# KlabCMU/KinPoly

Hardware: AMD Instinct MI355X
Metric: env-steps/sec (whole node) at 4096 envs/GPU, 69-DoF SMPL (higher is better)
Workload: dtype f32

## Files before the change

### include/kinpoly_sim.h

```cpp
#ifndef KINPOLY_SIM_H
#define KINPOLY_SIM_H
#include <stdint.h>
#ifdef __cplusplus
extern "C" {
#endif

typedef struct kp_model kp_model;
typedef struct kp_sim kp_sim;

#define KP_NQ 76
#define KP_NV 75
#define KP_NU 69
#define KP_NBODY 24
#define KP_CC_OBS_DIM 784
#define KP_AR_OBS_DIM 105
#define KP_AR_OBS_DIM_NO_ACTION 101
#define KP_KIN_ACTION_DIM 80
#define KP_CC_ACTION_DIM 75

kp_model* kp_model_load(const char* kpm_path);
int kp_model_compile(const char* xml_path, const char* uhc_yml_path, const char* out_kpm_path);
kp_model* kp_model_load_xml(const char* xml_path, const char* uhc_yml_path);
void kp_model_free(kp_model*);
int kp_model_set_option(kp_model*, const char* name, double value);
double kp_model_get_option(const kp_model*, const char* name);

kp_sim* kp_sim_create(const kp_model*, int n_envs, int device_id, void* hip_stream);
void kp_sim_destroy(kp_sim*);
int kp_sim_n_envs(const kp_sim*);

int kp_sim_set_stream(kp_sim*, void* hip_stream);

const uint32_t* kp_sim_status_device(kp_sim*);

int kp_sim_contacts(kp_sim*, float* out_host);

int kp_sim_mass_matrix(kp_sim*, float* M, float* bias);

int kp_sim_set_state(kp_sim*, const float* qpos, const float* qvel, const uint8_t* env_mask);

int kp_sim_set_target(kp_sim*, const float* target_qpos, const uint8_t* env_mask);

int kp_sim_set_objects(kp_sim*, const float* obj_qpos, const uint8_t* env_mask);

int kp_sim_fk(kp_sim*, int n_rows, const float* qpos, float* qpos_out, float* wbpos, float* wbquat, float* bquat, float* body_com);

int kp_sim_pose_contacts(kp_sim*, int n_rows, const float* xpos, const float* xquat, const float* obj_qpos, float pen_margin,
                         float* pen, int32_t* ncon, uint32_t* hits);

int kp_model_hull_planes(const kp_model*, float* planes4, int32_t* adr);

typedef struct { float figure[4][3], object[3], floor[2][3], sky[3], zfar; } kp_render_style;
void kp_render_style_default(kp_render_style*);

int kp_sim_render(kp_sim*, int n_rows, int n_fig, const float* xpos, const float* xquat, const float* obj_qpos, const float* camera, int camera_rows,
                  int width, int height, const kp_render_style* style, int32_t* geom, float* depth, uint8_t* rgba);

int kp_sim_render_ego(kp_sim*, int n_rows, int n_fig, const float* xpos, const float* xquat, const float* obj_qpos, const float* camera,
                      const float* xpos_b, const float* xquat_b, const float* obj_qpos_b, const float* camera_b, int camera_rows, int width, int height,
                      int hide_body, const kp_render_style* style, int grid_x, int grid_y,
                      int32_t* geom, float* depth, uint8_t* rgba, float* flow, uint8_t* ok, float* cells);

int kp_sim_fk_backward(kp_sim*, int n_rows, const float* qpos, const float* wbpos, const float* wbquat, const float* grad_wbpos, float* grad_qpos);

int kp_sim_step_ctrl(kp_sim*, const float* cc_action, int n_substeps, const uint8_t* env_mask);

int kp_sim_step_kin(kp_sim*, const float* kin_action, float* next_qpos);

int kp_sim_step_head(kp_sim*, const float* kin_action);

int kp_sim_obs_cc(kp_sim*, float* out, const float* zf_mean, const float* zf_std, float clip);

int kp_sim_obs_cc_ex(kp_sim*, float* out, const float* zf_mean, const float* zf_std, float clip, const float* phase);
int kp_sim_cc_obs_dim(const kp_sim*);

typedef struct {
    int T;
    const float* head_pose;
    const float* head_vels;
    const float* obj_head_relative_poses;
    const float* action_one_hot;
    const float* gt_bquat;
    const float* gt_wbpos;
    const float* obj_qpos;
    const int32_t* cur_t;
    const int32_t* row;
} kp_ctx;

int kp_sim_step_begin(kp_sim*);

int kp_sim_obs_ar(kp_sim*, const kp_ctx* ctx, float* out);
int kp_sim_ar_obs_dim(const kp_sim*);

typedef struct {
    float w_hp, w_hq, w_p, w_jp, w_act_p, w_act_v;
    float k_hp, k_hq, k_p, k_jp, k_act_p, k_act_v;
    float dt;
    float body_diff_thresh;
    float body_diff_gt_thresh;
    int use_gt_term;
} kp_reward_cfg;
int kp_sim_term_reward(kp_sim*, const kp_ctx* ctx, const kp_reward_cfg* cfg, float* reward, float* info, uint8_t* fail, float* diffs);

int kp_sim_post_step(kp_sim*, const kp_ctx* ctx, const kp_reward_cfg* cfg, int32_t* cur_t, const int32_t* row_len, int env_episode_len,
                     float* reward, float* info, uint8_t* fail, float* diffs, uint8_t* done, uint8_t* end, float* percent, int32_t* done_count, float* obj7);

typedef struct {
    float w_hp, w_hq, w_p, w_v, w_e;
    float k_hp, k_hq, k_p, k_v, k_e;
    float dt, body_diff_thresh, body_diff_gt_thresh;
    int use_gt_term;
    const float* b_diffw;
} kp_reward_cfg_v2;
int kp_sim_term_reward_v2(kp_sim*, const kp_ctx* ctx, const kp_reward_cfg_v2* cfg, float* reward, float* info, uint8_t* fail, float* diffs);
int kp_sim_post_step_v2(kp_sim*, const kp_ctx* ctx, const kp_reward_cfg_v2* cfg, int32_t* cur_t, const int32_t* row_len, int env_episode_len,
                        float* reward, float* info, uint8_t* fail, float* diffs, uint8_t* done, uint8_t* end, float* percent, int32_t* done_count, float* obj7);

int kp_sim_reset_rows(kp_sim*, const float* init_qpos, const float* init_qvel, const int32_t* row, const uint8_t* env_mask, int32_t* cur_t, int set_target,
                      float* aux_rows, int aux_cols, const float* row_obj_qpos, const float* row_action_one_hot, float* obj7);

int kp_pool_advance(int n, int n_slots, const uint8_t* done, int32_t* head, int32_t* ahead, int32_t* row, void* hip_stream);

typedef struct {
    int n, T, t, ctx_T;
    const float* obs; const uint8_t* fresh; const float* qpos; const float* ctx_qpos; const int32_t* row; const int32_t* cur_t; const int32_t* row_len; const float* row_meta;
    float* states; uint8_t* episode_start; float* curr_qpos; float* gt_target_qpos; float* meta;
} kp_record_pre;
typedef struct {
    int n, T, t; float fr_num;
    const float* action; const float* reward; const uint8_t* fail; const uint8_t* done; const float* percent; const float* c_info;
    const float* obs; const float* qpos; const float* cc_action; const float* cc_state; const float* meta;
    float* actions; float* rewards; uint8_t* fails; uint8_t* dones; float* percents; float* c_infos;
    float* next_states; float* res_qpos; float* cc_actions; float* cc_states; float* v_metas;
} kp_record_post;
int kp_rollout_record_pre(const kp_record_pre*, void* hip_stream);
int kp_rollout_record_post(const kp_record_post*, void* hip_stream);
int kp_rollout_record_pre_w(const kp_record_pre*, int obs_dim, void* hip_stream);
int kp_rollout_record_post_w(const kp_record_post*, int obs_dim, void* hip_stream);

int kp_gae(int n_envs, int T, const float* rewards, const float* masks, const float* values, float gamma, float tau,
           float* advantages, float* returns, void* hip_stream);
int kp_gae_bootstrap(int n_envs, int T, const float* rewards, const float* masks, const float* values, const float* last_values,
                     float gamma, float tau, float* advantages, float* returns, void* hip_stream);

int kp_mcp_compose(int n, int K, int A, const float* logits, const float* prim, const float* noise, int noise_stride, const float* stdv, float* out, void* hip_stream);

int kp_kin_advance(int n, const float* qpos, const float* kin_action, float dt, float* next_qpos, float* qvel_fd, void* hip_stream);

int kp_mcp_tail(int n, int K, int J, int A, const float* h2, const float* b2, const float* w3, int ldw, const float* b3, const float* logits, const float* noise,
                int noise_stride, const float* stdv, float* out, void* hip_stream);

int kp_gru_cell_step(int n, int H, int D, const float* gi, const float* gh, const float* b_ih, const float* b_hh, const float* h_in, const float* state,
                     float* h_out, float* xcat, void* hip_stream);

// ... 168 lines not shown
```

### kinpoly_amd/csrc/kp_obs_kernels.hpp

```cpp
#pragma once
#include "kp_quat.hpp"

namespace kp {

__global__ void k_step_kin(int n, const float* __restrict__ qpos, const float* __restrict__ act, float* __restrict__ next_qpos, float dt) {
    int e = blockIdx.x * blockDim.x + threadIdx.x;
    if (e >= n) return;
    const float* q = qpos + (size_t)e * D_NQ;
    const float* a = act + (size_t)e * 80;
    float* o = next_qpos + (size_t)e * D_NQ;
    Q4 rot = Q4{q[3], q[4], q[5], q[6]};
    Q4 hq = q_heading(rot);
    V3 linv = q_mul_vec(hq, v3(a[74], a[75], a[76]));
    o[0] = q[0] + linv.x * dt; o[1] = q[1] + linv.y * dt;
    o[2] = a[0];
    V3 angv = q_mul_vec(rot, v3(a[77], a[78], a[79]));
    Q4 nr = qmul(q_from_expmap(dt * angv), rot);
    o[3] = nr.w; o[4] = nr.x; o[5] = nr.y; o[6] = nr.z;
    for (int j = 0; j < D_NU; j++) o[7 + j] = a[5 + j];
}

__global__ void k_kin_advance(int n, const float* __restrict__ qpos, const float* __restrict__ act, float dt, float* __restrict__ next_qpos, float* __restrict__ qvel) {
    int e = blockIdx.x * blockDim.x + threadIdx.x;
    if (e >= n) return;
    const float* q = qpos + (size_t)e * D_NQ;
    const float* a = act + (size_t)e * 80;
    float* o = next_qpos + (size_t)e * D_NQ;
    float* v = qvel + (size_t)e * D_NV;
    const Q4 rot = Q4{q[3], q[4], q[5], q[6]};
    const Q4 hq = q_heading(rot);
    const V3 linv = q_mul_vec(hq, v3(a[74], a[75], a[76]));
    const float nx = q[0] + linv.x * dt, ny = q[1] + linv.y * dt, nz = a[0];
    const V3 angv = q_mul_vec(rot, v3(a[77], a[78], a[79]));
    Q4 nr = qmul(q_from_expmap(dt * angv), rot);
    const float nn = sqrtf(nr.w * nr.w + nr.x * nr.x + nr.y * nr.y + nr.z * nr.z);
    nr = Q4{nr.w / nn, nr.x / nn, nr.y / nn, nr.z / nn};
    o[0] = nx; o[1] = ny; o[2] = nz; o[3] = nr.w; o[4] = nr.x; o[5] = nr.y; o[6] = nr.z;
    const float idt = 1.0f / dt;
    v[0] = (nx - q[0]) * idt; v[1] = (ny - q[1]) * idt; v[2] = (nz - q[2]) * idt;
    const float c2 = rot.w * rot.w + rot.x * rot.x + rot.y * rot.y + rot.z * rot.z;
    const Q4 qrel = qmul(nr, Q4{rot.w / c2, -rot.x / c2, -rot.y / c2, -rot.z / c2});
    float sn = sqrtf(qrel.x * qrel.x + qrel.y * qrel.y + qrel.z * qrel.z);
    const V3 ev = dt * angv;
    const bool small = !(sn > 0.0f) || (ev.x == 0.0f && ev.y == 0.0f && ev.z == 0.0f);
    sn = fmaxf(sn, 1e-30f);
    const V3 axis = small ? v3(1.f, 0.f, 0.f) : v3(qrel.x / sn, qrel.y / sn, qrel.z / sn);
    float angle = small ? 0.0f : 2.0f * atan2f(sn, qrel.w);
    if (angle > KP_PI) angle -= KP_2PI;
    if (angle < -KP_PI) angle += KP_2PI;
    const V3 rv = (angle * idt) * axis;
    const float cn = sqrtf(c2);
    const float qw = rot.w / cn;
    const V3 u = v3(-rot.x / cn, -rot.y / cn, -rot.z / cn);
    const V3 t = 2.0f * cross(u, rv);
    const V3 wv = rv + qw * t + cross(u, t);
    v[3] = wv.x; v[4] = wv.y; v[5] = wv.z;
    for (int j = 0; j < D_NU; j++) { const float nj = a[5 + j]; o[7 + j] = nj; v[6 + j] = (nj - q[7 + j]) * idt; }
}

struct TargetBufs { float *qpos, *wbpos, *wbquat, *bquat, *com; };
struct KinStep { const float *act, *xpos, *xquat; float *prev_bquat, *prev_hpos; float dt; };
__global__ __launch_bounds__(256) void k_target_fk(int n, const float* __restrict__ tq, const uint8_t* __restrict__ mask, TargetBufs B,
                                                    const float* __restrict__ body_pos, const float* __restrict__ body_ipos, const int8_t* __restrict__ parent,
                                                    const uint8_t* __restrict__ depth, KinStep K = KinStep{nullptr, nullptr, nullptr, nullptr, nullptr, 0.f}) {
    __shared__ float sq[4][80], swq[4][D_NB * 4], swp[4][D_NB * 3];
    const int w = threadIdx.x >> 6, lane = threadIdx.x & 63;
    const int e = blockIdx.x * 4 + w;
    const bool live = e < n && !(mask && !mask[e]);
    if (!__syncthreads_or(live)) return;
    if (live) {
        const float* q = tq + (size_t)e * D_NQ;
        if (K.act) {
            const float* a = K.act + (size_t)e * 80;
            if (lane < D_NB) {
                const Q4 r = lane == 0 ? Q4{q[3], q[4], q[5], q[6]} : q_euler_sxyz(q[7 + 3 * (lane - 1)], q[8 + 3 * (lane - 1)], q[9 + 3 * (lane - 1)]);
                float* o = K.prev_bquat + ((size_t)e * D_NB + lane) * 4;
                o[0] = r.w; o[1] = r.x; o[2] = r.y; o[3] = r.z;
                if (lane == 13) {
                    for (int k = 0; k < 3; k++) K.prev_hpos[(size_t)e * 7 + k] = K.xpos[(size_t)e * 72 + 39 + k];
                    for (int k = 0; k < 4; k++) K.prev_hpos[(size_t)e * 7 + 3 + k] = K.xquat[(size_t)e * 96 + 52 + k];
                }
            }
            if (lane == 32) {
                const Q4 rot = Q4{q[3], q[4], q[5], q[6]};
                const V3 linv = q_mul_vec(q_heading(rot), v3(a[74], a[75], a[76]));
                const V3 angv = q_mul_vec(rot, v3(a[77], a[78], a[79]));
                const Q4 nr = qmul(q_from_expmap(K.dt * angv), rot);
                sq[w][0] = q[0] + linv.x * K.dt; sq[w][1] = q[1] + linv.y * K.dt; sq[w][2] = a[0];
                sq[w][3] = nr.w; sq[w][4] = nr.x; sq[w][5] = nr.y; sq[w][6] = nr.z;
            }
            for (int j = lane; j < D_NU; j += 64) sq[w][7 + j] = a[5 + j];
        } else {
            for (int i = lane; i < D_NQ; i += 64) sq[w][i] = q[i];
        }
    }
    __syncthreads();
    const int b = lane;
    Q4 wqb = Q4{1.f, 0.f, 0.f, 0.f}, lq = wqb, bq = wqb;
    V3 pos = v3(0.f, 0.f, 0.f);
    int dep = 99, p = 0;
    if (live && b < D_NB) {
        dep = depth[b]; p = parent[b] < 0 ? 0 : parent[b];
        const float* q = sq[w];
        if (b == 0) {
            Q4 rq = Q4{q[3], q[4], q[5], q[6]};
            const float rn = sqrtf(rq.w * rq.w + rq.x * rq.x + rq.y * rq.y + rq.z * rq.z);
            rq = Q4{rq.w / rn, rq.x / rn, rq.y / rn, rq.z / rn};
            wqb = rq; bq = rq; pos = v3(q[0], q[1], q[2]);
        } else {
            const float* ang = q + 7 + 3 * (b - 1);
            lq = q_euler_rzyx(ang[0], ang[1], ang[2]);
            bq = q_euler_sxyz(ang[0], ang[1], ang[2]);
        }
    }
    for (int lev = 0; lev < D_NLEV; lev++) {
        if (dep == lev) {
            if (b > 0) {
                const Q4 pq = Q4{swq[w][4 * p], swq[w][4 * p + 1], swq[w][4 * p + 2], swq[w][4 * p + 3]};
                pos = q_mul_vec(pq, ld3(body_pos + 3 * b)) + ld3(swp[w] + 3 * p);
                wqb = qmul(pq, lq);
            }
            swq[w][4 * b] = wqb.w; swq[w][4 * b + 1] = wqb.x; swq[w][4 * b + 2] = wqb.y; swq[w][4 * b + 3] = wqb.z;
            st3(swp[w] + 3 * b, pos);
        }
        __syncthreads();
    }
    if (live && b < D_NB) {
        if (B.bquat) { float* o = B.bquat + (size_t)e * 96 + 4 * b; o[0] = bq.w; o[1] = bq.x; o[2] = bq.y; o[3] = bq.z; }
        if (B.wbpos) st3(B.wbpos + (size_t)e * 72 + 3 * b, pos);
        if (B.wbquat) { float* o = B.wbquat + (size_t)e * 96 + 4 * b; o[0] = wqb.w; o[1] = wqb.x; o[2] = wqb.y; o[3] = wqb.z; }
        if (B.com) st3(B.com + (size_t)e * 72 + 3 * b, q_mul_vec(wqb, ld3(body_ipos + 3 * b)) + pos);
    }
    if (live && B.qpos) {
        float* oq = B.qpos + (size_t)e * D_NQ;
        for (int i = lane; i < D_NQ; i += 64) oq[i] = (i >= 3 && i < 7) ? swq[w][i - 3] : sq[w][i];
    }
}

__global__ __launch_bounds__(256) void k_fk_wbpos_grad(int n, const float* __restrict__ qpos, const float* __restrict__ wbpos, const float* __restrict__ wbquat,
                                                        const float* __restrict__ gw, float* __restrict__ gq, const int8_t* __restrict__ parent,
                                                        const uint8_t* __restrict__ subtree) {
    __shared__ float sp[4][D_NB * 3], sg[4][D_NB * 3];
    const int w = threadIdx.x >> 6, b = threadIdx.x & 63;
    const int e = blockIdx.x * 4 + w;
    const bool live = e < n;
    if (live && b < D_NB) {
        st3(sp[w] + 3 * b, ld3(wbpos + (size_t)e * 72 + 3 * b));
        st3(sg[w] + 3 * b, ld3(gw + (size_t)e * 72 + 3 * b));
    }
    __syncthreads();
    if (!live || b >= D_NB) return;
    const V3 pb = ld3(sp[w] + 3 * b);
    V3 F = v3(0.f, 0.f, 0.f), M = v3(0.f, 0.f, 0.f);
    const int nb = subtree[b];
    for (int j = b + 1; j < b + nb; j++) {
        const V3 g = ld3(sg[w] + 3 * j);
        F = F + g; M = M + cross(ld3(sp[w] + 3 * j) - pb, g);
    }
    const float* q = qpos + (size_t)e * D_NQ;
    float* o = gq + (size_t)e * D_NQ;
    if (b == 0) {
        st3(o, F + ld3(sg[w]));
        const float qn = sqrtf(q[3] * q[3] + q[4] * q[4] + q[5] * q[5] + q[6] * q[6]);
        const float* uq = wbquat + (size_t)e * 96;
        const Q4 G = qmul(Q4{0.f, 2.f * M.x, 2.f * M.y, 2.f * M.z}, Q4{uq[0], uq[1], uq[2], uq[3]});
        o[3] = G.w / qn; o[4] = G.x / qn; o[5] = G.y / qn; o[6] = G.z / qn;
    } else {
        const int p = parent[b];
        const float* pq = wbquat + (size_t)e * 96 + 4 * p;
        float R[9];
        q_matrix(Q4{pq[0], pq[1], pq[2], pq[3]}, R);
        const float tz = q[7 + 3 * (b - 1)], ty = q[8 + 3 * (b - 1)];
        float sz, cz, sy, cy;
        sincosf(tz, &sz, &cz); sincosf(ty, &sy, &cy);
        const V3 az = mulmat(R, v3(0.f, 0.f, 1.f));
        const V3 ay = mulmat(R, v3(-sz, cz, 0.f));
        const V3 ax = mulmat(R, v3(cz * cy, sz * cy, -sy));
        o[7 + 3 * (b - 1)] = dot(az, M); o[8 + 3 * (b - 1)] = dot(ay, M); o[9 + 3 * (b - 1)] = dot(ax, M);
    }
}

__global__ void k_bquat(int n, const float* __restrict__ qpos, float* __restrict__ out) {
    int t = blockIdx.x * blockDim.x + threadIdx.x;
    if (t >= n * D_NB) return;
    int e = t / D_NB, b = t - e * D_NB;
    const float* q = qpos + (size_t)e * D_NQ;
    Q4 r;
    if (b == 0) r = Q4{q[3], q[4], q[5], q[6]};
    else r = q_euler_sxyz(q[7 + 3 * (b - 1)], q[8 + 3 * (b - 1)], q[9 + 3 * (b - 1)]);
    float* o = out + (size_t)t * 4;
    o[0] = r.w; o[1] = r.x; o[2] = r.y; o[3] = r.z;
}

struct ObsCcArgs {
    int n;
    const float *qpos, *qvel, *xpos, *xquat, *xipos;
    const float *t_qpos, *t_wbpos, *t_wbquat, *t_com;
    float br_inv[4];
    const float *zf_mean, *zf_std; float clip;
    float* out;
};
template <int V, bool VROOT, bool HEAD, bool DEHEAD, bool PHASE>
struct ObsCcLayout {
    static constexpr int LV = VROOT ? 6 : 75;
    static constexpr int D = V == 0 ? (HEAD ? 1 : 0) + 74 + LV + 69 + (PHASE ? 1 : 0) : 229 + LV + (V == 1 ? 4 : 2) * 72 + 2 * 96;
};
template <int V, bool VROOT, bool HEAD, bool DEHEAD, bool PHASE>
__device__ __forceinline__ void obs_cc_body(const ObsCcArgs& A, const float* __restrict__ phase) {
    using L = ObsCcLayout<V, VROOT, HEAD, DEHEAD, PHASE>;
    constexpr int LV = L::LV, D = L::D;
    __shared__ float ob[D];
    const int e = blockIdx.x, tid = threadIdx.x;
    if (e >= A.n) return;
    const float* qpos = A.qpos + (size_t)e * D_NQ;
    const float* qvel = A.qvel + (size_t)e * D_NV;
    const float* tq = A.t_qpos + (size_t)e * D_NQ;
    const Q4 rq = Q4{qpos[3], qpos[4], qpos[5], qpos[6]};
    if constexpr (V == 0) {
        constexpr int H = HEAD ? 1 : 0, K = H + 74 + LV;
        if (tid == 0) {
            if (HEAD) ob[0] = heading_angle(rq);
            const Q4 r = DEHEAD ? qmul(q_inverse(q_heading(rq)), rq) : rq;
            ob[H] = qpos[2]; ob[H + 1] = r.w; ob[H + 2] = r.x; ob[H + 3] = r.y; ob[H + 4] = r.z;
            const V3 v = q_tmul_vec(rq, v3(qvel[0], qvel[1], qvel[2]));
            ob[H + 74] = v.x; ob[H + 75] = v.y; ob[H + 76] = v.z;
            if (PHASE) ob[K + 69] = phase[e];
        }
        for (int i = tid; i < 69; i += 64) { ob[H + 5 + i] = qpos[7 + i]; ob[K + i] = tq[7 + i]; }
        for (int i = tid; i < LV - 3; i += 64) ob[H + 77 + i] = qvel[3 + i];
    } else {
        constexpr int P = 229 + LV, NJ = V == 1 ? 4 : 2, Q = P + 72 * NJ;
        const Q4 binv = Q4{A.br_inv[0], A.br_inv[1], A.br_inv[2], A.br_inv[3]};
        const Q4 crq = qmul(rq, binv);
        const Q4 hq = q_heading(crq);
        const Q4 trq = qmul(Q4{tq[3], tq[4], tq[5], tq[6]}, binv);
        const V3 root = v3(qpos[0], qpos[1], qpos[2]);
        if (tid == 0) {
            ob[0] = hq.w; ob[1] = hq.x; ob[2] = hq.y; ob[3] = hq.z;
            Q4 dh = qmul(q_inverse(hq), crq);
            ob[78] = qpos[2]; ob[79] = dh.w; ob[80] = dh.x; ob[81] = dh.y; ob[82] = dh.z;
            Q4 dq = qmul(trq, q_inverse(crq));
            ob[152] = tq[2] - qpos[2]; ob[153] = dq.w; ob[154] = dq.x; ob[155] = dq.y; ob[156] = dq.z;
            V3 v = q_tmul_vec(crq, q_tmul_vec(rq, v3(qvel[0], qvel[1], qvel[2])));
            ob[226] = v.x; ob[227] = v.y; ob[228] = v.z;
            float rel_h = heading_angle(trq) - heading_angle(crq);
            if (rel_h > KP_PI) rel_h -= KP_2PI;
            if (rel_h < -KP_PI) rel_h += KP_2PI;
            ob[P - 3] = rel_h;
            V3 rp = q_tmul_vec(crq, v3(trq.w, trq.x, trq.y) - root);
            ob[P - 2] = rp.x; ob[P - 1] = rp.y;
        }
        for (int i = tid; i < 74; i += 64) ob[4 + i] = tq[2 + i];
        for (int i = tid; i < 69; i += 64) { ob[83 + i] = qpos[7 + i]; ob[157 + i] = tq[7 + i] - qpos[7 + i]; }
        for (int i = tid; i < LV - 3; i += 64) ob[229 + i] = qvel[3 + i];
        if (tid < D_NB) {
            const int b = tid;
            const float* xp = A.xpos + (size_t)e * 72 + 3 * b;
            const float* xi = A.xipos + (size_t)e * 72 + 3 * b;
            const float* xq = A.xquat + (size_t)e * 96;
            V3 cj = ld3(xp), ci = ld3(xi);
            V3 tj = ld3(A.t_wbpos + (size_t)e * 72 + 3 * b), tc = ld3(A.t_com + (size_t)e * 72 + 3 * b);
            V3 p1 = q_tmul_vec(crq, cj - root), p2 = q_tmul_vec(crq, tj - cj), p3 = q_tmul_vec(crq, ci - root), p4 = q_tmul_vec(crq, tc - ci);
            ob[P + b] = p1.x; ob[P + 24 + b] = p1.y; ob[P + 48 + b] = p1.z;
            ob[P + 72 + b] = p2.x; ob[P + 96 + b] = p2.y; ob[P + 120 + b] = p2.z;
            if (V == 1) {
                ob[P + 144 + b] = p3.x; ob[P + 168 + b] = p3.y; ob[P + 192 + b] = p3.z;
                ob[P + 216 + b] = p4.x; ob[P + 240 + b] = p4.y; ob[P + 264 + b] = p4.z;
            }
            const float* twq = A.t_wbquat + (size_t)e * 96 + 4 * b;
            Q4 tqt = Q4{twq[0], twq[1], twq[2], twq[3]};
            Q4 cq = (xq[0] == 0.f) ? tqt : Q4{xq[4 * b], xq[4 * b + 1], xq[4 * b + 2], xq[4 * b + 3]};
            Q4 r1 = qmul(q_inverse(hq), cq), r2 = qmul(q_inverse(cq), tqt);
            float* o1 = ob + Q + 4 * b; o1[0] = r1.w; o1[1] = r1.x; o1[2] = r1.y; o1[3] = r1.z;
            float* o2 = ob + Q + 96 + 4 * b; o2[0] = r2.w; o2[1] = r2.x; o2[2] = r2.y; o2[3] = r2.z;
        }
    }
    __syncthreads();
    for (int i = tid; i < D; i += 64) {
        float v = ob[i];
        if (A.zf_mean) {
            v = (v - A.zf_mean[i]) / (A.zf_std[i] + 1e-8f);
            if (A.clip > 0.f) v = fminf(fmaxf(v, -A.clip), A.clip);
        }
        A.out[(size_t)e * D + i] = v;
    }
}
template <int V, bool VROOT, bool HEAD, bool DEHEAD, bool PHASE>
__global__ __launch_bounds__(64) void k_obs_cc(ObsCcArgs A, const float* __restrict__ phase) { obs_cc_body<V, VROOT, HEAD, DEHEAD, PHASE>(A, phase); }
__global__ __launch_bounds__(64) void k_obs_cc_uhc(ObsCcArgs A) { obs_cc_body<1, false, false, false, false>(A, nullptr); }

}
```

### kinpoly_amd/csrc/kp_rollout_kernels.hpp

```cpp
#pragma once
#include "kp_obs_kernels.hpp"
#include "kp_obs_ar_row.hpp"

namespace kp {

__device__ __forceinline__ int obj_action_start(const float* one_hot) {
    if (!one_hot) return -1;
    int a = -1;
    for (int k = 0; k < 4; k++) if (a < 0 && one_hot[k] != 0.f) a = k;
    return a < 0 ? -1 : (a == 0 ? 0 : (a == 1 ? 7 : (a == 2 ? 21 : 28)));
}

template <bool VEL, bool HEAD, bool ACTION>
__global__ __launch_bounds__(256) void k_obs_ar(int n, CtxDev C, const float* __restrict__ qpos, const float* __restrict__ qvel,
                                                 const float* __restrict__ xpos, const float* __restrict__ xquat, float* __restrict__ out) {
    const int l = threadIdx.x & 31, e = blockIdx.x * 8 + (threadIdx.x >> 5);
    if (e >= n) return;
    obs_ar_row<VEL, HEAD, ACTION>(C, e, l, qpos, qvel, xpos, xquat, out + (size_t)e * ObsArLayout<VEL, HEAD, ACTION>::D);
}

template <bool ACTION>
__global__ void k_obs_ar_thread(int n, CtxDev C, const float* __restrict__ qpos, const float* __restrict__ xpos, const float* __restrict__ xquat,
                                float* __restrict__ out) {
    int e = blockIdx.x * blockDim.x + threadIdx.x;
// ... 88 lines not shown
    float pq = 0.f, pp = 0.f, pg = 0.f, vel2 = 0.f, bd = 0.f, bgd = 0.f;
    if (b < D_NB) {
        const Q4 cb = b == 0 ? Q4{q[3], q[4], q[5], q[6]} : q_euler_sxyz(q[7 + 3 * (b - 1)], q[8 + 3 * (b - 1)], q[9 + 3 * (b - 1)]);
        const float* tb = t_bquat + (size_t)e * 96 + 4 * b;
        if constexpr (RV == 1) pq = quat_norm_v2(qmul(cb, q_inverse(Q4{tb[0], tb[1], tb[2], tb[3]})));
        const V3 x = ld3(xp + 3 * b);
        const V3 dpos = x - ld3(t_wbpos + (size_t)e * 72 + 3 * b);
        pp = sqrtf(dot(dpos, dpos));
        const float wgt = diffw ? diffw[b] : 1.0f;
        bd = wgt * pp;
        const V3 dg = x - ld3(gtw + 3 * b);
        bgd = wgt * sqrtf(dot(dg, dg));
        const Q4 g = Q4{gtb[4 * b], gtb[4 * b + 1], gtb[4 * b + 2], gtb[4 * b + 3]};
        const Q4 gpv = Q4{gtp[4 * b], gtp[4 * b + 1], gtp[4 * b + 2], gtp[4 * b + 3]};
        if constexpr (RV == 1) pg = quat_norm_v2(qmul(g, q_inverse(cb)));
        else {
            const Q4 qd = qmul(cb, q_inverse(g));
            const float pa = atan2f(sqrtf(qd.x * qd.x + qd.y * qd.y + qd.z * qd.z), qd.w) * W.b_diffw[b];
            pq = pa * pa;
            pg = dot(dg, dg);
        }
        const float* pb = prev_bquat + (size_t)e * 96 + 4 * b;
        constexpr float rot_eps = RV == 1 ? 1e-8f : 1e-6f;
        const V3 cv = (1.0f / W.dt) * rot_from_quat(qmul(cb, q_inverse(Q4{pb[0], pb[1], pb[2], pb[3]})), rot_eps);
        const V3 gv = (1.0f / W.dt) * rot_from_quat(qmul(g, q_inverse(gpv)), rot_eps);
        const V3 dv = cv - gv;
        vel2 = dot(dv, dv);
    }
#pragma unroll
    for (int m = 16; m >= 1; m >>= 1) {
        pq += __shfl_xor(pq, m, 32); pp += __shfl_xor(pp, m, 32); pg += __shfl_xor(pg, m, 32);
        vel2 += __shfl_xor(vel2, m, 32); bd += __shfl_xor(bd, m, 32); bgd += __shfl_xor(bgd, m, 32);
    }
    if (b != 0 || !valid) return;
    const float* xq = xquat + (size_t)e * 96;
    const float* hp = C.head_pose + (C.r(e) * C.T + t) * 7;
    const V3 hd = ld3(xp + 39) - ld3(hp);
    const float hp_r = expf(-W.k_hp * dot(hd, hd));
    const Q4 hq = qmul(Q4{xq[52], xq[53], xq[54], xq[55]}, q_inverse(Q4{hp[3], hp[4], hp[5], hp[6]}));
    const float hqd = quat_norm_v2(hq);
    const float hq_r = expf(-W.k_hq * hqd * hqd);
    if constexpr (RV == 1) {
        pq *= (1.0f / 24.0f); pp *= (1.0f / 24.0f); pg *= (1.0f / 24.0f);
        const float p_r = expf(-W.k_p * pq * pq), jp_r = expf(-W.k_jp * pp * pp);
        const float gt_r = expf(-W.k_act_p * pg), av_r = expf(-W.k_act_v * vel2);
        reward[e] = W.w_hp * hp_r + W.w_hq * hq_r + W.w_p * p_r + W.w_jp * jp_r + W.w_act_p * gt_r + W.w_act_v * av_r;
        float* inf = info + (size_t)e * 6;
        inf[0] = hp_r; inf[1] = hq_r; inf[2] = p_r; inf[3] = jp_r; inf[4] = gt_r; inf[5] = av_r;
    } else {
        const float p_r = expf(-W.k_p * pq), v_r = expf(-W.k_v * vel2), e_r = expf(-W.k_e * pg);
        reward[e] = W.w_hp * hp_r + W.w_hq * hq_r + W.w_p * p_r + W.w_v * v_r + W.w_e * e_r;
        float* inf = info + (size_t)e * 6;
        inf[0] = hp_r; inf[1] = hq_r; inf[2] = p_r; inf[3] = v_r; inf[4] = e_r; inf[5] = 0.f;
    }
    const bool failed = (bd > W.thresh) || (W.use_gt && bgd > W.gt_thresh) || !(bd == bd);
    fail[e] = failed;
    diffs[2 * e] = bd; diffs[2 * e + 1] = bgd;
    if (POST) {
        const int clen = PS.row_len[C.r(e)];
        const bool ended = t_now >= (clen < PS.episode_len ? clen : PS.episode_len);
        PS.cur_t[e] = t_now;
        PS.end[e] = ended; PS.done[e] = failed || ended;
        PS.percent[e] = (float)t_now / (float)clen;
        if (PS.done_count && (failed || ended)) atomicAdd(PS.done_count, 1);
        if (PS.obj7) {
            const int st = obj_action_start(C.action_one_hot + C.r(e) * 4);
            if (st >= 0) for (int k = 0; k < 7; k++) PS.obj7[(size_t)e * 7 + k] = PS.sim_obj_qpos[(size_t)e * 35 + st + k];
        }
    }
}

__global__ void k_reset_rows(int n, const float* __restrict__ init_qpos, const float* __restrict__ init_qvel, const int* __restrict__ row,
                             const uint8_t* __restrict__ mask, int* __restrict__ cur_t, float* __restrict__ qpos, float* __restrict__ qvel,
                             float* __restrict__ qpos_d, float* __restrict__ qvel_d, float* __restrict__ warm, float* __restrict__ aux_rows, int aux_cols) {
    const int e = blockIdx.x, i = threadIdx.x;
    if (e >= n || (mask && !mask[e])) return;
    for (int c = i; c < aux_cols; c += 128) aux_rows[(size_t)e * aux_cols + c] = 0.f;
    const size_t r = row ? (size_t)row[e] : (size_t)e;
    if (i < D_NQ) { const float v = init_qpos[r * D_NQ + i]; qpos[(size_t)e * D_NQ + i] = v; qpos_d[(size_t)e * D_NQ + i] = v; }
    if (i < D_NV) { const float v = init_qvel[r * D_NV + i]; qvel[(size_t)e * D_NV + i] = v; qvel_d[(size_t)e * D_NV + i] = v; warm[(size_t)e * D_NV + i] = 0.f; }
    if (i == 0 && cur_t) cur_t[e] = 0;
}

__global__ void k_pool_advance(int n, int n_slots, const uint8_t* __restrict__ done, int* __restrict__ head, int* __restrict__ ahead, int* __restrict__ row) {
    const int e = blockIdx.x * blockDim.x + threadIdx.x;
    if (e >= n || !done[e]) return;
    const int a = ahead[e];
    ahead[e] = a - 1;
    if (a <= 0) return;
    int h = head[e] + 1;
    if (h >= n_slots) h = 0;
    head[e] = h;
    row[e] = h * n + e;
}

struct RecordPre {
    int n, T, t, ctx_T, obs_dim;
    const float* obs; const uint8_t* fresh; const float* qpos; const float* ctx_qpos; const int* row; const int* cur_t; const int* row_len; const float* row_meta;
    float* states; uint8_t* episode_start; float* curr_qpos; float* gt_target_qpos; float* meta;
};
struct RecordPost {
    int n, T, t, obs_dim; float fr_num;
    const float* action; const float* reward; const uint8_t* fail; const uint8_t* done; const float* percent; const float* c_info;
    const float* obs; const float* qpos; const float* cc_action; const float* cc_state; const float* meta_t;
    float* actions; float* rewards; uint8_t* fails; uint8_t* dones; float* percents; float* c_infos;
    float* next_states; float* res_qpos; float* cc_actions; float* cc_states; float* v_metas;
};

__device__ __forceinline__ void copy_row(float* __restrict__ dst, const float* __restrict__ src, int dim) {
    for (int i = threadIdx.x; i < dim; i += blockDim.x) dst[i] = src[i];
}

__global__ void k_record_pre(RecordPre R) {
    const int e = blockIdx.x;
    if (e >= R.n) return;
    const size_t at = (size_t)e * R.T + R.t;
    if (R.states) copy_row(R.states + at * R.obs_dim, R.obs + (size_t)e * R.obs_dim, R.obs_dim);
    if (R.curr_qpos) copy_row(R.curr_qpos + at * 76, R.qpos + (size_t)e * 76, 76);
    const int r = R.row ? R.row[e] : e;
    if (R.gt_target_qpos) {
        int f = R.cur_t[e] + 1;
        const int last = R.row_len[r];
        if (f > last) f = last;
        copy_row(R.gt_target_qpos + at * 76, R.ctx_qpos + ((size_t)r * R.ctx_T + f) * 76, 76);
    }
    if (threadIdx.x == 0) {
        if (R.episode_start) R.episode_start[at] = R.fresh[e];
        if (R.meta) { R.meta[at * 2] = R.row_meta[(size_t)r * 2]; R.meta[at * 2 + 1] = R.row_meta[(size_t)r * 2 + 1]; }
    }
}

__global__ void k_record_post(RecordPost R) {
    const int e = blockIdx.x;
    if (e >= R.n) return;
    const size_t at = (size_t)e * R.T + R.t;
    if (R.actions) copy_row(R.actions + at * 80, R.action + (size_t)e * 80, 80);
    if (R.next_states) copy_row(R.next_states + at * R.obs_dim, R.obs + (size_t)e * R.obs_dim, R.obs_dim);
    if (R.res_qpos) copy_row(R.res_qpos + at * 76, R.qpos + (size_t)e * 76, 76);
    if (R.cc_actions) copy_row(R.cc_actions + at * 75, R.cc_action + (size_t)e * 75, 75);
    if (R.cc_states) copy_row(R.cc_states + at * 784, R.cc_state + (size_t)e * 784, 784);
    if (R.c_infos && threadIdx.x < 6) R.c_infos[at * 6 + threadIdx.x] = R.c_info[(size_t)e * 6 + threadIdx.x];
    if (threadIdx.x == 0) {
        if (R.rewards) R.rewards[at] = R.reward[e];
        if (R.fails) R.fails[at] = R.fail[e];
        if (R.dones) R.dones[at] = R.done[e];
        if (R.percents) R.percents[at] = R.percent[e];
        if (R.v_metas) { R.v_metas[at * 3] = R.meta_t[at * 2]; R.v_metas[at * 3 + 1] = R.meta_t[at * 2 + 1]; R.v_metas[at * 3 + 2] = R.fr_num; }
    }
}

__global__ void k_gae(int n, int T, const float* __restrict__ rewards, const float* __restrict__ masks, const float* __restrict__ values,
                      const float* __restrict__ last_values, float gamma, float tau, float* __restrict__ adv, float* __restrict__ ret) {
    int e = blockIdx.x * blockDim.x + threadIdx.x;
    if (e >= n) return;
    float prev_v = last_values ? last_values[e] : 0.f, prev_a = 0.f;
    for (int t = T - 1; t >= 0; t--) {
        size_t i = (size_t)e * T + t;
        float m = masks[i], v = values[i];
        float delta = rewards[i] + gamma * prev_v * m - v;
        float a = delta + gamma * tau * prev_a * m;
        adv[i] = a; ret[i] = v + a;
        prev_v = v; prev_a = a;
    }
}

__global__ void k_mcp_compose(int n, int K, int A, const float* __restrict__ logits, const float* __restrict__ prim, const float* __restrict__ noise,
// ... 53 lines not shown
```

### kinpoly_amd/csrc/kp_sim.hip

```cpp
#include <hip/hip_runtime.h>

#include <climits>
#include <cmath>
#include <algorithm>
#include <array>
#include <cstdlib>
#include <cstring>
#include <cstdio>
#include <unistd.h>
#include <string>
#include <utility>
#include <vector>

#include "../../include/kinpoly_sim.h"
#include "kp_model.hpp"
#include "kp_obs_kernels.hpp"
#include "kp_rollout_kernels.hpp"
#include "kp_policy_kernels.hpp"
#include "kp_step_kernel.hpp"
#include "kp_readout.hpp"
#include "kp_pose_contacts.hpp"
#include "kp_render.hpp"
#include "kp_render_ego.hpp"
#include "kp_takes.hpp"
#include "kp_kin_tape.hpp"
#include "kp_obs_ctx.hpp"

namespace {
thread_local std::string g_err;
int fail(const std::string& m) { g_err = m; return -1; }
#define HIP_OK(expr) do { hipError_t e_ = (expr); if (e_ != hipSuccess) return fail(std::string(#expr) + ": " + hipGetErrorString(e_)); } while (0)
#define HIP_OK_NULL(expr) do { hipError_t e_ = (expr); if (e_ != hipSuccess) { fail(std::string(#expr) + ": " + hipGetErrorString(e_)); return nullptr; } } while (0)
int launched() { HIP_OK(hipGetLastError()); return 0; }
}

struct kp_model {
    kp::HostModel h;
    int contact = 1, limits = 1, stale = 1, solver_iter = 100, threads = 64, dynamic_objects = 1, lpt_order = -1, substeps_per_job = 4, queue_slots = 0, job_taper = 1, queue_fence = 1, queue_heavy = 160, queue_prio = -1, queue_late = -1, job_auto = 1, lean_queue = 1, lean_adaptive = 1, lds_pad = 0, lean_cap = kp::EnvLdsLean::MAXCON;
    double warm_extrap = -1.0;
    int planemesh_max = 3; double planemesh_tol = 0.3;
    int ar_obs_action = 1;
    int ar_obs_vel = 0, ar_obs_head = 1;
    int cc_obs_v = 1, cc_obs_vel_root = 0, cc_obs_heading = 0, cc_obs_deheading = 0, cc_obs_phase = 0;
    int cc_action_v = 1, cc_rfc = 1, cc_meta_pd = 0;
    int actuation = 1;
    double solver_tol = 1e-8, gravity_z = -9.81, gravity_x = 0.0, gravity_y = 0.0;
};

struct StateRows {
    float *qpos = nullptr, *qvel = nullptr, *qpos_d = nullptr, *qvel_d = nullptr, *warm = nullptr, *warm2 = nullptr, *warm3 = nullptr;
    float *xpos = nullptr, *xquat = nullptr, *xipos = nullptr, *prev_bquat = nullptr, *prev_hpos = nullptr;
    int* diag = nullptr;
};
struct JobQueue {
    int* order = nullptr; unsigned* cost = nullptr;
    unsigned *jobq = nullptr, *jobctr = nullptr, *ovfq = nullptr;
    float* spd_next = nullptr;
    int wave_slots = 2048;
    int nsub = -1, layout = -1;
};
struct OverflowReadback {
    unsigned* host = nullptr; hipEvent_t ev[2] = {nullptr, nullptr}; bool pending[2] = {false, false};
    long lean_off_until = -1; int fallbacks = 0;
    unsigned last = 0;
};
struct ObjectRows {
    float *qpos = nullptr, *geoms = nullptr;
    float *qvel = nullptr, *warm = nullptr, *warm2 = nullptr;
    signed char* slot = nullptr;
    int* ngeom = nullptr;
    const float* d_geoms = nullptr; const float* d_mass = nullptr; int n_geoms = 0, n_obj = 0;
    bool on = false;
};
struct Timing {
    hipEvent_t ev0 = nullptr, ev1 = nullptr, last0 = nullptr, last1 = nullptr;
    std::vector<hipEvent_t> ring;
    int ring_used = 0;
    bool ring_on = false, timed = false;
};

struct RenderTables {
    const float* planes = nullptr; const int32_t* adr = nullptr;
    float* partial = nullptr; size_t partial_n = 0;
};

struct InvDynScratch {
    float* buf = nullptr; size_t rows = 0;
};

struct MarkerScratch {
    static constexpr int MAXK = 1024, WORDS = 4 * MAXK + 25;
    void* buf = nullptr;
    std::vector<uint32_t> host;
};

struct kp_sim {
    const kp_model* model = nullptr;
    int n = 0, device = 0;
    int ar_obs_vel = 0, ar_obs_head = 1, ar_obs_action = 1;
    int ar_obs_dim = KP_AR_OBS_DIM;
    int cc_obs_v = 1, cc_obs_vel_root = 0, cc_obs_heading = 0, cc_obs_deheading = 0, cc_obs_phase = 0, cc_obs_dim = KP_CC_OBS_DIM;
    kp::XcArgs xc{KP_CC_ACTION_DIM, 0, 1, 0};
    bool xc_on = false;
    hipStream_t stream = nullptr;
    std::vector<void*> allocs;
    kp::DevTables T{};
    kp::Params P{};
    float* diffw = nullptr;
    StateRows st;
    kp::TargetBufs tgt{};
    JobQueue q;
    OverflowReadback ovf;
    ObjectRows obj;
    RenderTables rd;
    InvDynScratch idyn;
    MarkerScratch mk;
    Timing tm;
    long launch_index = 0;
    int last_nsub = 15;
    unsigned long long* prof = nullptr;
    bool prof_noted = false;
    float* dbg_contacts = nullptr;
    int32_t* uhc_stage = nullptr;
};

struct kp_takes {
    const kp_model* model = nullptr;
    int device = 0;
    kp::TakeTables L{};
    float* obj = nullptr;
    std::vector<int32_t> off;
    std::vector<void*> allocs;
};

namespace {

template <typename T, typename S>
const T* upload(kp_sim* s, const std::vector<S>& src, bool* ok) {
    std::vector<T> tmp(src.size());
    for (size_t i = 0; i < src.size(); i++) tmp[i] = (T)src[i];
    void* d = nullptr;
    if (hipMalloc(&d, std::max<size_t>(sizeof(T) * tmp.size(), 16)) != hipSuccess) { *ok = false; return nullptr; }
    s->allocs.push_back(d);
    if (hipMemcpy(d, tmp.data(), sizeof(T) * tmp.size(), hipMemcpyHostToDevice) != hipSuccess) { *ok = false; return nullptr; }
    return (const T*)d;
}

float* dalloc(kp_sim* s, size_t count, bool* ok) {
    void* d = nullptr;
    if (hipMalloc(&d, sizeof(float) * count) != hipSuccess) { *ok = false; return nullptr; }
    s->allocs.push_back(d);
    hipMemset(d, 0, sizeof(float) * count);
    return (float*)d;
}

bool build_tables(kp_sim* s) {
    const kp::HostModel& m = s->model->h;
    using namespace kp;
    bool ok = true;
    auto& T = s->T;
    T.body_pos = upload<float>(s, m.body_pos, &ok); T.body_ipos = upload<float>(s, m.body_ipos, &ok);
    T.body_mass = upload<float>(s, m.body_mass, &ok); T.body_inertia = upload<float>(s, m.body_inertia, &ok);
    T.body_rbound = upload<float>(s, m.body_rbound, &ok); T.mesh_rbound = upload<float>(s, m.mesh_rbound, &ok);
    std::vector<double> invw(NB), liminvw(NU), lo(NU), hi(NU);
    for (int b = 0; b < NB; b++) invw[b] = m.body_invweight0[2 * b];
    for (int j = 0; j < NU; j++) { liminvw[j] = m.dof_invweight0[6 + j]; lo[j] = m.jnt_range[2 * j]; hi[j] = m.jnt_range[2 * j + 1]; }
    T.body_invw = upload<float>(s, invw, &ok); T.lim_invw = upload<float>(s, liminvw, &ok);
    T.jnt_lo = upload<float>(s, lo, &ok); T.jnt_hi = upload<float>(s, hi, &ok);
    T.dof_armature = upload<float>(s, m.dof_armature, &ok);
    T.kp = upload<float>(s, m.kp, &ok); T.kd = upload<float>(s, m.kd, &ok); T.tlim = upload<float>(s, m.torque_lim, &ok);
    T.ascale = upload<float>(s, m.a_scale, &ok);
    s->diffw = const_cast<float*>(upload<float>(s, m.body_diffw, &ok));
    T.verts = upload<float>(s, m.verts, &ok);
    T.vert_adr = upload<uint16_t>(s, m.vert_adr, &ok);
    T.vert_nbr_adr = upload<uint16_t>(s, m.vert_nbr_adr, &ok); T.vert_nbr = upload<uint8_t>(s, m.vert_nbr, &ok);
    T.dof_body = upload<uint8_t>(s, m.dof_body, &ok);
    T.body_parent = upload<int8_t>(s, m.body_parent, &ok); T.body_depth = upload<uint8_t>(s, m.body_depth, &ok);
    T.body_subtree = upload<uint8_t>(s, m.body_subtree, &ok); T.jnt_limited = upload<uint8_t>(s, m.jnt_limited, &ok);
    for (int b = 1; b < NB; b++) {
        if (m.body_parent[b] >= b) return false;
        for (int j = 0; j < 3; j++) if (m.dof_body[6 + 3 * (b - 1) + j] != b) return false;
    }
    for (int b = 0; b < NB; b++)
        for (int k = b + 1; k < NB; k++) {
            bool desc = false;
            for (int p = m.body_parent[k]; p >= 0; p = m.body_parent[p]) if (p == b) desc = true;
            if (desc != (k < b + m.body_subtree[b])) return false;
        }
    std::vector<int> lev_start(D_NLEV + 2, 0), lev_body;
    for (int lev = 0; lev <= D_NLEV; lev++) {
        lev_start[lev] = (int)lev_body.size();
        for (int b = 0; b < NB; b++) if (m.body_depth[b] == lev) lev_body.push_back(b);
    }
    lev_start[D_NLEV + 1] = (int)lev_body.size();
    if ((int)lev_body.size() != NB || lev_start[D_NLEV] != NB) return false;
// ... 62 lines not shown
    P.mu = (float)o[OPT_FRIC]; P.margin = (float)o[OPT_MARGIN];
    P.pm_max = s->model->planemesh_max; P.pm_tol = (float)s->model->planemesh_tol;
    P.scale = (float)(1.0 / (o[OPT_MEANINERTIA] * (o.size() > OPT_NV_FULL ? o[OPT_NV_FULL] : NV)));
    P.rfc_scale = (float)o[OPT_RFC_SCALE]; P.rfc_lim = (float)o[OPT_RFC_LIM];
    double bn = o[OPT_BR_W] * o[OPT_BR_W] + o[OPT_BR_X] * o[OPT_BR_X] + o[OPT_BR_Y] * o[OPT_BR_Y] + o[OPT_BR_Z] * o[OPT_BR_Z];
    P.br_inv[0] = (float)(o[OPT_BR_W] / bn); P.br_inv[1] = (float)(-o[OPT_BR_X] / bn);
    P.br_inv[2] = (float)(-o[OPT_BR_Y] / bn); P.br_inv[3] = (float)(-o[OPT_BR_Z] / bn);
    P.tol = (float)s->model->solver_tol; P.max_iter = s->model->solver_iter;
    P.contact = s->model->contact; P.limits = s->model->limits; P.stale = s->model->stale; P.actuation = s->model->actuation;
    return ok;
}

int job_schedule(int nsub, int spj, int taper, int* sizes) {
    int parts = 0, rem = nsub, size = spj;
    while (rem > 0 && parts < 16) {
        int take = parts == 15 ? rem : std::min(rem, size);
        if (rem - take > 0 && rem - take < spj) take = rem;
        sizes[parts++] = take; rem -= take;
        size += taper;
    }
    std::reverse(sizes, sizes + parts);
    return parts;
}

bool lean_eligible(const kp_sim& s) { return !s.obj.on && s.model->lean_queue && s.model->threads == 64 && s.P.stale && !s.xc_on; }

int envs_per_cu(size_t lds_bytes, int reg_cap) { return std::min(reg_cap, 128 / (int)((lds_bytes + 1279) / 1280)); }

int poll_overflow(kp_sim* s) {
    for (int k = 0; k < 2; k++) {
        if (!s->ovf.pending[k]) continue;
        const hipError_t e = hipEventQuery(s->ovf.ev[k]);
        if (e == hipErrorNotReady) continue;
        s->ovf.pending[k] = false;
        if (e != hipSuccess) return fail(std::string("hipEventQuery(ovf_ev): ") + hipGetErrorString(e));
        s->ovf.last = s->ovf.host[k];
        if ((size_t)s->ovf.host[k] * 64 > (size_t)s->n) { s->ovf.lean_off_until = s->launch_index + 64; s->ovf.fallbacks++; }
    }
    return 0;
}

enum Layout { FULL = 0, OBJECTS = 1, LEAN = 2 };
struct StepPlan {
    bool queue, lpt;
    bool prof_per_env;
    Layout layout;
    int threads, slots, parts, sizes[16], queue_prio, queue_late, ovf_grid;
    size_t lds;
};

StepPlan plan_step(const kp_sim& s, int nsub, bool capturing) {
    const kp_model& m = *s.model;
    StepPlan p{};
    bool lean = lean_eligible(s);
    if (lean && nsub > 0 && s.ovf.host && !capturing && m.lean_adaptive && s.launch_index < s.ovf.lean_off_until) lean = false;
    p.layout = s.obj.on ? OBJECTS : lean ? LEAN : FULL;
    p.threads = m.threads;
    p.lpt = nsub > 0 && (m.lpt_order > 0 || (m.lpt_order < 0 && s.obj.on));
    const size_t lds = s.obj.on ? sizeof(kp::EnvLdsObj) : sizeof(kp::EnvLds);
    size_t lds_q = lean ? sizeof(kp::EnvLdsLean) : lds;
    if (m.lds_pad > 0) lds_q = std::max(lds_q, (size_t)m.lds_pad);
    p.slots = m.queue_slots > 0 ? m.queue_slots : s.q.wave_slots / 8 * envs_per_cu(lds_q, lean ? 12 : 8);
    const bool lean_auto = lean && m.job_auto;
    const int spj = lean_auto ? 5 : m.substeps_per_job, taper = lean_auto ? 0 : m.job_taper;
    if (spj > 0 && nsub > 0) {
        p.parts = job_schedule(nsub, spj, taper, p.sizes);
        if (const char* e = std::getenv("KP_JOB_SCHEDULE")) {
            int tmp[16], np = 0, sum = 0;
            for (const char* c = e; *c && np < 16;) { tmp[np] = std::atoi(c); sum += tmp[np++]; while (*c && *c != ',') c++; if (*c) c++; }
            if (sum == nsub) { p.parts = np; std::copy(tmp, tmp + np, p.sizes); }
        }
    }
    const int resident_full = s.q.wave_slots / 8 * envs_per_cu(lds, 8);
    const bool queue = nsub > 0 && p.parts > 1 && m.threads == 64 && s.n > std::min(p.slots, resident_full) && s.n <= 0xFFFFFF;
    p.queue = queue && !s.prof; p.prof_per_env = queue && s.prof;
    p.lds = p.queue ? lds_q : lds;
    p.queue_prio = m.queue_prio >= 0 ? m.queue_prio : (lean ? 3 : 0);
    p.queue_late = m.queue_late >= 0 ? m.queue_late : (lean ? 1 : 0);
    p.ovf_grid = std::min(std::min(s.n, resident_full), std::max(128, 2 * (int)std::min<unsigned>(s.ovf.last, 1u << 20)));
    return p;
}

template <int NT, bool OBJ>
void launch_per_env(const kp_sim* s, const kp::StepArgs& A, int nsub, size_t lds) {
    if (nsub > 0 && s->prof && s->xc_on) hipLaunchKernelGGL((kp::kp_step_kernel_xc<NT, OBJ, true>), dim3(s->n), dim3(NT), lds, s->stream, A, s->xc);
    else if (nsub > 0 && s->prof) hipLaunchKernelGGL((kp::kp_step_kernel<NT, OBJ, true>), dim3(s->n), dim3(NT), lds, s->stream, A);
    else if (nsub > 0 && s->xc_on) hipLaunchKernelGGL((kp::kp_step_kernel_xc<NT, OBJ>), dim3(s->n), dim3(NT), lds, s->stream, A, s->xc);
    else if (nsub > 0) hipLaunchKernelGGL((kp::kp_step_kernel<NT, OBJ>), dim3(s->n), dim3(NT), lds, s->stream, A);
    else hipLaunchKernelGGL((kp::kp_forward_kernel<NT, OBJ>), dim3(s->n), dim3(NT), lds, s->stream, A);
}

int timing_begin(kp_sim* s, hipEvent_t* e0, hipEvent_t* e1) {
    Timing& t = s->tm;
    *e0 = t.ev0; *e1 = t.ev1;
    if (t.ring_on && t.ring_used < 4096) {
        if ((int)t.ring.size() < 2 * (t.ring_used + 1)) {
            hipEvent_t a, b;
            HIP_OK(hipEventCreate(&a)); HIP_OK(hipEventCreate(&b));
            t.ring.push_back(a); t.ring.push_back(b);
        }
        *e0 = t.ring[2 * t.ring_used]; *e1 = t.ring[2 * t.ring_used + 1];
        t.ring_used++;
    }
    HIP_OK(hipEventRecord(*e0, s->stream));
    return 0;
}
int timing_end(kp_sim* s, hipEvent_t e0, hipEvent_t e1) {
    HIP_OK(hipEventRecord(e1, s->stream));
    s->tm.last0 = e0; s->tm.last1 = e1; s->tm.timed = true;
    return 0;
}

kp::StepArgs step_args(const kp_sim* s, const StepPlan& p, int nsub, const float* action, const uint8_t* mask, const float* base_qpos) {
    const kp_model& m = *s->model;
    const StateRows& st = s->st; const ObjectRows& o = s->obj; const JobQueue& q = s->q;
    kp::StepArgs A{};
    A.T = s->T; A.P = s->P; A.n_envs = s->n; A.n_substeps = nsub;
    A.qpos = st.qpos; A.qvel = st.qvel; A.qpos_d = st.qpos_d; A.qvel_d = st.qvel_d; A.warm = st.warm; A.warm2 = st.warm2; A.warm3 = st.warm3;
    A.target_qpos = base_qpos ? base_qpos : s->tgt.qpos; A.action = action; A.env_mask = mask;
    A.xpos = st.xpos; A.xquat = st.xquat; A.xipos = st.xipos; A.diag = st.diag; A.prof = s->prof; A.dbg_contacts = s->dbg_contacts;
    A.geoms = o.geoms; A.ngeom = o.ngeom; A.obj_slot = o.slot; A.obj_qpos = o.qpos; A.obj_qvel = o.qvel; A.obj_warm = o.warm; A.obj_warm2 = o.warm2;
    A.warm_extrap = m.warm_extrap < 0 ? (o.on ? 0.75f : 0.f) : (float)m.warm_extrap;
    A.order = p.lpt ? q.order : nullptr; A.order_valid = p.lpt; A.cost = q.cost;
    A.jobq = q.jobq; A.jobctr = q.jobctr; A.ovfq = q.ovfq; A.spd_next = q.spd_next; A.lean_cap = m.lean_cap;
    A.n_parts = p.queue ? p.parts : 1; A.queue_fence = m.queue_fence; A.queue_heavy = m.queue_heavy; A.queue_prio = p.queue_prio; A.queue_late = p.queue_late;
    for (int k = 0; p.queue && k < p.parts; k++) (k < 8 ? A.part_sub_lo : A.part_sub_hi) |= (unsigned long long)(p.sizes[k] & 255) << (8 * (k & 7));
    return A;
}

int launch_queue(kp_sim* s, const StepPlan& p, kp::StepArgs& A, int nsub, bool capturing) {
    JobQueue& q = s->q;
    if (nsub != q.nsub || (int)p.layout != q.layout) {
        HIP_OK(hipMemsetAsync(q.jobctr + 32, 0, 2 * sizeof(unsigned), s->stream));
        q.nsub = nsub; q.layout = (int)p.layout;
    }
    const unsigned total = (unsigned)s->n * (unsigned)p.parts;
    hipLaunchKernelGGL(kp::k_queue_init, dim3((total + 255) / 256), dim3(256), 0, s->stream, s->n, total, q.jobq, q.jobctr, A.order);
    A.order = nullptr;
    if (s->xc_on && p.layout == OBJECTS) hipLaunchKernelGGL((kp::kp_step_queue_kernel_xc<true>), dim3(p.slots), dim3(64), p.lds, s->stream, A, s->xc);
    else if (s->xc_on) hipLaunchKernelGGL((kp::kp_step_queue_kernel_xc<false>), dim3(p.slots), dim3(64), p.lds, s->stream, A, s->xc);
    else if (p.layout == OBJECTS) hipLaunchKernelGGL((kp::kp_step_queue_kernel<true>), dim3(p.slots), dim3(64), p.lds, s->stream, A);
    else if (p.layout == FULL) hipLaunchKernelGGL((kp::kp_step_queue_kernel<false>), dim3(p.slots), dim3(64), p.lds, s->stream, A);
    else {
        hipLaunchKernelGGL((kp::kp_step_queue_kernel<false, true>), dim3(p.slots), dim3(64), p.lds, s->stream, A);
        hipLaunchKernelGGL(kp::kp_step_overflow_kernel, dim3(p.ovf_grid), dim3(64), sizeof(kp::EnvLds), s->stream, A);
        const int k = (int)(s->launch_index & 1);
        if (s->ovf.host && !capturing && !s->ovf.pending[k]) {
            HIP_OK(hipMemcpyAsync(s->ovf.host + k, q.jobctr + 64, sizeof(unsigned), hipMemcpyDeviceToHost, s->stream));
            HIP_OK(hipEventRecord(s->ovf.ev[k], s->stream));
            s->ovf.pending[k] = true;
        }
    }
    return 0;
}

int launch_step(kp_sim* s, const float* action, int nsub, const uint8_t* mask, bool time_it, const float* base_qpos = nullptr) {
    const int threads = s->model->threads;
    if (s->obj.on && threads != 64) return fail("object contact needs threads_per_env = 64");
    if (threads != 64 && threads != 128 && threads != 256) return fail("threads_per_env must be 64, 128 or 256");
    hipStreamCaptureStatus cap = hipStreamCaptureStatusNone;
    const bool capturing = hipStreamIsCapturing(s->stream, &cap) == hipSuccess && cap != hipStreamCaptureStatusNone;
    time_it = time_it && !capturing;
    hipEvent_t e0 = nullptr, e1 = nullptr;
    if (time_it && timing_begin(s, &e0, &e1)) return -1;
    if (nsub > 0 && s->ovf.host && !capturing && lean_eligible(*s) && poll_overflow(s)) return -1;
    const StepPlan p = plan_step(*s, nsub, capturing);
    if (nsub > 0) { s->launch_index++; s->last_nsub = nsub; }
    if (p.prof_per_env && !s->prof_noted) {
        std::fprintf(stderr, "kp_sim: KP_PROFILE=1: the job-queue kernels carry no phase profiler; this handle's control steps run one workgroup per env "
                             "(kp_step_kernel), whose profiling instantiation fills kp_sim_phase_cycles\n");
        s->prof_noted = true;
    }
    kp::StepArgs A = step_args(s, p, nsub, action, mask, base_qpos);
    if (p.lpt) hipLaunchKernelGGL(kp::k_lpt_order, dim3(1), dim3(1024), 0, s->stream, s->n, s->q.cost, s->q.order);
    if (p.queue) { if (launch_queue(s, p, A, nsub, capturing)) return -1; }
    else if (s->obj.on) launch_per_env<64, true>(s, A, nsub, p.lds);
    else if (p.threads == 64) launch_per_env<64, false>(s, A, nsub, p.lds);
    else if (p.threads == 128) launch_per_env<128, false>(s, A, nsub, p.lds);
    else launch_per_env<256, false>(s, A, nsub, p.lds);
    HIP_OK(hipGetLastError());
    return time_it ? timing_end(s, e0, e1) : 0;
}

void launch_target_fk(const kp_sim* s, int n, const float* tq, const uint8_t* mask, const kp::TargetBufs& B,
                      const kp::KinStep& K = kp::KinStep{nullptr, nullptr, nullptr, nullptr, nullptr, 0.f}) {
    hipLaunchKernelGGL(kp::k_target_fk, dim3((n + 3) / 4), dim3(256), 0, s->stream, n, tq, mask, B, s->T.body_pos, s->T.body_ipos, s->T.body_parent, s->T.body_depth, K);
}

}

extern "C" {

const char* kp_last_error(void) { return g_err.c_str(); }
const char* kp_version(void) { return "kinpoly_sim 0.1 (gfx950)"; }

kp_model* kp_model_load(const char* path) {
    kp_model* m = new kp_model();
    if (!kp::load_kpm(path, m->h)) { fail("kp_model_load: " + m->h.error); delete m; return nullptr; }
    m->gravity_z = m->h.opt[kp::OPT_GZ]; m->gravity_x = m->h.opt[kp::OPT_GX]; m->gravity_y = m->h.opt[kp::OPT_GY];
    m->solver_tol = m->h.opt[kp::OPT_SOLVER_TOL];
    m->solver_iter = (int)m->h.opt[kp::OPT_SOLVER_ITER];
    if (m->solver_iter < 1) m->solver_iter = 100;
    m->planemesh_max = (int)m->h.planemesh[0]; m->planemesh_tol = m->h.planemesh[1];
    return m;
}
void kp_model_free(kp_model* m) { delete m; }

static int cc_action_width(int rfc, int meta) { return 69 + 6 * rfc + (meta == 1 ? 30 : meta == 2 ? 138 : 0); }

static int cc_obs_width(int v, int vel_root, int heading, int phase) {
    const int lv = vel_root ? 6 : 75;
    return v == 0 ? heading + 74 + lv + 69 + phase : 229 + lv + (v == 1 ? 4 : 2) * 72 + 2 * 96;
}

static int ar_obs_width(int vel, int head, int action) { return 74 + 75 * vel + 7 * head + 7 + 13 * head + 4 * action; }
static bool ar_obs_width_known(int d) {
    for (int k = 0; k < 8; k++) if (d == ar_obs_width(k & 1, (k >> 1) & 1, (k >> 2) & 1)) return true;
    return false;
}
#define KP_AR_OBS_WIDTHS "105, 101, 180, 176, 85, 81, 160 or 156"

enum OptRule { O_BOOL, O_TRI, O_INT, O_REAL, O_REAL32, O_ENUM, O_RANGE, O_CLAMP, O_THREADS, O_READ_ONLY };
struct Opt {
    const char* name;
    OptRule rule;
    int kp_model::*i; double kp_model::*d;
    double lo, hi;
    const char* must;
    bool clears_job_auto;
    double (*get)(const kp_model&);
};
constexpr double INF = HUGE_VAL;
#define OPT_I(name, rule, member, ...) Opt{name, rule, &kp_model::member, nullptr, __VA_ARGS__}
#define OPT_D(name, rule, member, ...) Opt{name, rule, nullptr, &kp_model::member, __VA_ARGS__}
#define OPT_RO(name, expr) Opt{name, O_READ_ONLY, nullptr, nullptr, 0, 0, nullptr, false, [](const kp_model& m) -> double { return expr; }}
static const Opt OPTIONS[] = {
    OPT_I("contact", O_BOOL, contact), OPT_I("limits", O_BOOL, limits), OPT_I("actuation", O_BOOL, actuation), OPT_I("stale_kinematics", O_BOOL, stale),
    OPT_D("gravity_z", O_REAL, gravity_z), OPT_D("gravity_x", O_REAL, gravity_x), OPT_D("gravity_y", O_REAL, gravity_y),
    OPT_I("solver_iter", O_INT, solver_iter), OPT_D("solver_tol", O_REAL, solver_tol), OPT_I("dynamic_objects", O_BOOL, dynamic_objects),
    OPT_I("planemesh_max", O_RANGE, planemesh_max, 1, 8), OPT_D("planemesh_tol", O_RANGE, planemesh_tol, 0, INF, ">= 0"),
    OPT_I("threads_per_env", O_THREADS, threads, 0, 0, "64, 128 or 256"),
    OPT_D("warm_extrap", O_REAL32, warm_extrap),
    OPT_I("ar_obs_action", O_ENUM, ar_obs_action, 0, 1, "1 (105-d observation with the action one-hot) or 0 (101-d, use_action: false)"),
    OPT_I("ar_obs_vel", O_ENUM, ar_obs_vel, 0, 1, "0 (no velocities) or 1 (use_vel: the 75 qvel follow the pose block)"),
    OPT_I("ar_obs_head", O_ENUM, ar_obs_head, 0, 1, "1 (with the head-tracking blocks) or 0 (use_head: false)"),
    OPT_RO("ar_obs_dim", ar_obs_width(m.ar_obs_vel, m.ar_obs_head, m.ar_obs_action)),
    OPT_I("cc_obs_v", O_ENUM, cc_obs_v, 0, 2, "0 (get_full_obs), 1 (get_full_obs_v1) or 2 (get_full_obs_v2)"),
    OPT_I("cc_obs_vel_root", O_ENUM, cc_obs_vel_root, 0, 1), OPT_I("cc_obs_heading", O_ENUM, cc_obs_heading, 0, 1),
    OPT_I("cc_obs_deheading", O_ENUM, cc_obs_deheading, 0, 1), OPT_I("cc_obs_phase", O_ENUM, cc_obs_phase, 0, 1),
    OPT_RO("cc_obs_dim", m.cc_obs_v == 0 ? cc_obs_width(0, m.cc_obs_vel_root, m.cc_obs_heading, m.cc_obs_phase) : cc_obs_width(m.cc_obs_v, m.cc_obs_vel_root, 0, 0)),
    OPT_I("cc_action_v", O_ENUM, cc_action_v, 0, 1), OPT_I("cc_rfc", O_ENUM, cc_rfc, 0, 1),
    OPT_I("cc_meta_pd", O_ENUM, cc_meta_pd, 0, 2, "0 (none), 1 (meta_pd: by substep) or 2 (meta_pd_joint: by joint)"),
    OPT_RO("cc_action_dim", cc_action_width(m.cc_rfc, m.cc_meta_pd)),
    OPT_RO("n_obj_geoms", (double)(m.h.obj_geoms.size() / 18)),
    OPT_RO("timestep", m.h.opt[kp::OPT_TIMESTEP]),
    OPT_I("lpt_order", O_TRI, lpt_order),
    OPT_I("substeps_per_job", O_RANGE, substeps_per_job, 0, 255, "0 (whole control step per workgroup) .. 255", true),
    OPT_I("job_taper", O_CLAMP, job_taper, 0, 8, nullptr, true),
    OPT_RO("job_auto", m.job_auto),
    OPT_I("queue_slots", O_RANGE, queue_slots, 0, INF, ">= 0 (0 = resident wave slots of the device)"),
    OPT_I("queue_fence", O_BOOL, queue_fence), OPT_I("queue_heavy", O_CLAMP, queue_heavy, 0, INT_MAX),
    OPT_I("queue_late", O_TRI, queue_late), OPT_I("queue_prio", O_CLAMP, queue_prio, -1, 3),
    OPT_I("lean_queue", O_BOOL, lean_queue), OPT_I("lean_adaptive", O_BOOL, lean_adaptive),
    OPT_I("lean_max_contacts", O_RANGE, lean_cap, 0, kp::EnvLdsLean::MAXCON),
    OPT_I("lds_pad", O_RANGE, lds_pad, 0, 65536, "0 .. 65536 bytes"),
    OPT_RO("lds_bytes_per_env", (double)sizeof(kp::EnvLds)), OPT_RO("lds_bytes_per_env_objects", (double)sizeof(kp::EnvLdsObj)),
    OPT_RO("lds_bytes_per_env_lean", (double)sizeof(kp::EnvLdsLean)),
};
#undef OPT_I
#undef OPT_D
#undef OPT_RO
static const Opt* find_option(const char* name) {
    for (const Opt& o : OPTIONS) if (name && !std::strcmp(name, o.name)) return &o;
    return nullptr;
}

int kp_model_set_option(kp_model* m, const char* name, double v) {
    if (!m || !name) return fail("kp_model_set_option: null argument");
    const Opt* o = find_option(name);
    if (!o || o->rule == O_READ_ONLY) return fail(std::string("kp_model_set_option: unknown option ") + name);
    bool ok = true;
    double x = v;
    switch (o->rule) {
        case O_BOOL: x = v != 0; break;
        case O_TRI: x = v < 0 ? -1 : (v != 0); break;
        case O_REAL32: x = (float)v; break;
        case O_ENUM: ok = false; for (int k = 0; k <= (int)o->hi; k++) ok = ok || v == k; break;
        case O_RANGE: ok = !(v < o->lo || v > o->hi); break;
        case O_CLAMP: x = std::max((int)o->lo, std::min((int)o->hi, (int)v)); break;
        case O_THREADS: ok = v == 64 || v == 128 || v == 256; break;
        default: break;
    }
    if (!ok) {
        const std::string must = o->must ? o->must : o->rule == O_ENUM ? "0 or 1" : std::to_string((int)o->lo) + " .. " + std::to_string((int)o->hi);
        return fail(std::string(name) + " must be " + must);
    }
    if (o->i) m->*(o->i) = (int)x; else m->*(o->d) = x;
    if (o->clears_job_auto) m->job_auto = 0;
    return 0;
}
double kp_model_get_option(const kp_model* m, const char* name) {
    const Opt* o = find_option(name);
    if (!m || !o) return NAN;
    return o->get ? o->get(*m) : o->i ? (double)(m->*(o->i)) : m->*(o->d);
}

kp_sim* kp_sim_create(const kp_model* m, int n_envs, int device_id, void* stream) {
    if (!m || n_envs <= 0) { fail("kp_sim_create: bad arguments"); return nullptr; }
    int ndev = 0;
    if (hipGetDeviceCount(&ndev) != hipSuccess || ndev == 0) { fail("kp_sim_create: no HIP device available (the simulator has no CPU fallback)"); return nullptr; }
    HIP_OK_NULL(hipSetDevice(device_id));
    kp_sim* s = new kp_sim();
    s->model = m; s->n = n_envs; s->device = device_id; s->stream = (hipStream_t)stream;
    s->ar_obs_vel = m->ar_obs_vel; s->ar_obs_head = m->ar_obs_head; s->ar_obs_action = m->ar_obs_action;
    s->ar_obs_dim = ar_obs_width(s->ar_obs_vel, s->ar_obs_head, s->ar_obs_action);
    s->cc_obs_v = m->cc_obs_v; s->cc_obs_vel_root = m->cc_obs_vel_root;
    s->cc_obs_heading = m->cc_obs_v == 0 && m->cc_obs_heading; s->cc_obs_deheading = m->cc_obs_v == 0 && m->cc_obs_deheading; s->cc_obs_phase = m->cc_obs_v == 0 && m->cc_obs_phase;
    s->cc_obs_dim = cc_obs_width(s->cc_obs_v, s->cc_obs_vel_root, s->cc_obs_heading, s->cc_obs_phase);
    s->xc = kp::XcArgs{cc_action_width(m->cc_rfc, m->cc_meta_pd), m->cc_action_v == 0, m->cc_rfc, m->cc_meta_pd};
    s->xc_on = m->cc_action_v != 1 || m->cc_rfc != 1 || m->cc_meta_pd != 0;
    bool ok = build_tables(s);
    const size_t N = n_envs;
    StateRows& st = s->st;
    st.qpos = dalloc(s, N * 76, &ok); st.qvel = dalloc(s, N * 75, &ok); st.qpos_d = dalloc(s, N * 76, &ok); st.qvel_d = dalloc(s, N * 75, &ok);
    st.warm = dalloc(s, N * 75, &ok); st.warm2 = dalloc(s, N * 75, &ok); st.warm3 = dalloc(s, N * 75, &ok);
    st.xpos = dalloc(s, N * 72, &ok); st.xquat = dalloc(s, N * 96, &ok); st.xipos = dalloc(s, N * 72, &ok);
    st.prev_bquat = dalloc(s, N * 96, &ok); st.prev_hpos = dalloc(s, N * 7, &ok); st.diag = (int*)dalloc(s, N * 4, &ok);
    s->tgt = kp::TargetBufs{dalloc(s, N * 76, &ok), dalloc(s, N * 72, &ok), dalloc(s, N * 96, &ok), dalloc(s, N * 96, &ok), dalloc(s, N * 72, &ok)};
    JobQueue& q = s->q;
    q.order = (int*)dalloc(s, N, &ok); q.cost = (unsigned*)dalloc(s, N, &ok);
    q.jobq = (unsigned*)dalloc(s, N * 16, &ok); q.jobctr = (unsigned*)dalloc(s, 128, &ok); q.ovfq = (unsigned*)dalloc(s, N, &ok);
    q.spd_next = dalloc(s, N * 80, &ok);
    hipDeviceProp_t prop;
    if (hipGetDeviceProperties(&prop, s->device) == hipSuccess && prop.multiProcessorCount > 0) q.wave_slots = prop.multiProcessorCount * 8;
    ObjectRows& o = s->obj;
    o.qpos = dalloc(s, N * 35, &ok); o.qvel = dalloc(s, N * 30, &ok); o.geoms = dalloc(s, N * kp::D_MAXGEOM * 17, &ok); o.ngeom = (int*)dalloc(s, N, &ok);
    o.warm = dalloc(s, N * 6 * kp::D_MAXOBJ, &ok); o.warm2 = dalloc(s, N * 6 * kp::D_MAXOBJ, &ok); o.slot = (signed char*)dalloc(s, (N * kp::D_MAXOBJ + 3) / 4 + 1, &ok);
    if (!m->h.obj_geoms.empty()) {
        o.d_geoms = upload<float>(s, m->h.obj_geoms, &ok); o.d_mass = upload<float>(s, m->h.obj_mass, &ok);
        o.n_geoms = (int)(m->h.obj_geoms.size() / 18); o.n_obj = (int)m->h.obj_mass.size();
    }
    if (const char* e = std::getenv("KP_PROFILE")) if (e[0] == '1') s->prof = (unsigned long long*)dalloc(s, N * 16, &ok);
    OverflowReadback& v = s->ovf;
    if (hipHostMalloc((void**)&v.host, 2 * sizeof(unsigned), hipHostMallocDefault) != hipSuccess) v.host = nullptr;
    else {
        v.host[0] = v.host[1] = 0u;
        if (hipEventCreateWithFlags(&v.ev[0], hipEventDisableTiming) != hipSuccess || hipEventCreateWithFlags(&v.ev[1], hipEventDisableTiming) != hipSuccess) { hipHostFree(v.host); v.host = nullptr; }
    }
    if (!ok || hipEventCreate(&s->tm.ev0) != hipSuccess || hipEventCreate(&s->tm.ev1) != hipSuccess) {
        fail("kp_sim_create: device allocation / table build failed");
        kp_sim_destroy(s);
        return nullptr;
    }
    return s;
}

void kp_sim_destroy(kp_sim* s) {
    if (!s) return;
    hipSetDevice(s->device);
    hipStreamSynchronize(s->stream);
    for (void* p : s->allocs) hipFree(p);
    if (s->rd.partial) hipFree(s->rd.partial);
    if (s->idyn.buf) hipFree(s->idyn.buf);
    if (s->mk.buf) hipFree(s->mk.buf);
    for (hipEvent_t e : s->tm.ring) hipEventDestroy(e);
    if (s->ovf.host) { hipHostFree(s->ovf.host); for (hipEvent_t e : s->ovf.ev) if (e) hipEventDestroy(e); }
    if (s->tm.ev0) hipEventDestroy(s->tm.ev0);
    if (s->tm.ev1) hipEventDestroy(s->tm.ev1);
    delete s;
}
int kp_sim_n_envs(const kp_sim* s) { return s ? s->n : -1; }

int kp_sim_set_stream(kp_sim* s, void* stream) {
    if (!s) return fail("kp_sim_set_stream: null argument");
    s->stream = (hipStream_t)stream;
    return 0;
}

const uint32_t* kp_sim_status_device(kp_sim* s) { return s ? s->q.jobctr : nullptr; }

int kp_sim_contacts(kp_sim* s, float* out_host) {
    if (!s) return fail("kp_sim_contacts: null argument");
    HIP_OK(hipSetDevice(s->device));
    const size_t count = (size_t)s->n * (1 + kp::D_MAXCON * 9);
    if (!s->dbg_contacts) {
        bool ok = true;
        s->dbg_contacts = dalloc(s, count, &ok);
        if (!ok) return fail("kp_sim_contacts: allocation failed");
        if (out_host) std::memset(out_host, 0, sizeof(float) * count);
        return 0;
    }
    if (!out_host) return 0;
    HIP_OK(hipStreamSynchronize(s->stream));
    HIP_OK(hipMemcpy(out_host, s->dbg_contacts, sizeof(float) * count, hipMemcpyDeviceToHost));
    return 0;
}

int kp_sim_mass_matrix(kp_sim* s, float* M, float* bias) {
    if (!s || (!M && !bias)) return fail("kp_sim_mass_matrix: null argument");
    HIP_OK(hipSetDevice(s->device));
    kp::StepArgs A{};
    A.T = s->T; A.P = s->P; A.n_envs = s->n; A.n_substeps = 0;
    A.qpos_d = s->st.qpos_d; A.qvel_d = s->st.qvel_d;
    hipLaunchKernelGGL(kp::kp_mass_kernel, dim3(s->n), dim3(64), sizeof(kp::EnvLds), s->stream, A, M, bias);
    return launched();
}

__global__ void k_copy_rows(int n, int dim, const float* __restrict__ src, float* __restrict__ dst, float* __restrict__ dst2,
                            const uint8_t* __restrict__ mask) {
    size_t t = (size_t)blockIdx.x * blockDim.x + threadIdx.x;
    if (t >= (size_t)n * dim) return;
    int e = (int)(t / dim);
    if (mask && !mask[e]) return;
    float v = src ? src[t] : 0.f;
    dst[t] = v;
    if (dst2) dst2[t] = v;
}
static void copy_rows(const kp_sim* s, int dim, const float* src, float* dst, float* dst2, const uint8_t* mask) {
    hipLaunchKernelGGL(k_copy_rows, dim3((s->n * dim + 255) / 256), dim3(256), 0, s->stream, s->n, dim, src, dst, dst2, mask);
}

int kp_sim_set_state(kp_sim* s, const float* qpos, const float* qvel, const uint8_t* mask) {
    if (!s || !qpos || !qvel) return fail("kp_sim_set_state: null argument");
    HIP_OK(hipSetDevice(s->device));
    copy_rows(s, 76, qpos, s->st.qpos, s->st.qpos_d, mask);
    copy_rows(s, 75, qvel, s->st.qvel, s->st.qvel_d, mask);
    copy_rows(s, 75, nullptr, s->st.warm, nullptr, mask);
    HIP_OK(hipGetLastError());
    return launch_step(s, nullptr, 0, mask, false);
}

int kp_sim_set_target(kp_sim* s, const float* tq, const uint8_t* mask) {
    if (!s || !tq) return fail("kp_sim_set_target: null argument");
    HIP_OK(hipSetDevice(s->device));
    launch_target_fk(s, s->n, tq, mask, s->tgt);
    return launched();
}

__global__ void k_set_objects(int n, const float* __restrict__ obj_qpos_all, const uint8_t* __restrict__ mask, float* __restrict__ obj_qpos,
                              float* __restrict__ geoms, int* __restrict__ ngeom, const float* __restrict__ og, const float* __restrict__ omass,
                              int n_og, int n_obj, int dynamic, signed char* __restrict__ slot, float* __restrict__ obj_qvel, float* __restrict__ obj_warm,
                              const int* __restrict__ row, const float* __restrict__ one_hot, float* __restrict__ obj7) {
    int e = blockIdx.x * blockDim.x + threadIdx.x;
    if (e >= n) return;
    if (mask && !mask[e]) return;
    int ng = 0, ns = 0;
    const size_t r = row ? (size_t)row[e] : (size_t)e;
    const float* src = obj_qpos_all + r * 35;
// ... 404 lines not shown
        if (!ok) { s->uhc_stage = nullptr; return fail("kp_sim_uhc_assign: allocation failed"); }
    }
    kp::UhcAssignArgs A{};
    if (take_ids) {
        HIP_OK(hipMemcpyAsync(s->uhc_stage, take_ids, sizeof(int32_t) * s->n, hipMemcpyHostToDevice, s->stream));
        A.take_ids = s->uhc_stage;
        if (start) { HIP_OK(hipMemcpyAsync(s->uhc_stage + s->n, start, sizeof(int32_t) * s->n, hipMemcpyHostToDevice, s->stream)); A.start = s->uhc_stage + s->n; }
    }
    A.L = t->L; A.n = s->n; A.keep_t = keep_t; A.obs_v = c->obs_v; A.st = *st; A.mask = mask; A.noise = noise; A.a_ref = c->a_ref;
    A.qpos = s->st.qpos; A.qpos_d = s->st.qpos_d; A.qvel = s->st.qvel; A.qvel_d = s->st.qvel_d; A.warm = s->st.warm;
    A.t_qpos = s->tgt.qpos; A.t_wbpos = s->tgt.wbpos; A.t_wbquat = s->tgt.wbquat; A.t_bquat = s->tgt.bquat; A.t_com = s->tgt.com;
    if (t->obj) {
        ObjectRows& o = s->obj;
        kp::UhcAssignObjArgs B{};
        B.A = A; B.obj_tab = t->obj; B.obj_qpos = o.qpos; B.obj_qvel = o.qvel; B.obj_warm = o.warm; B.geoms = o.geoms; B.ngeom = o.ngeom; B.slot = o.slot;
        B.og = o.d_geoms; B.omass = o.d_mass; B.n_og = o.n_geoms; B.n_obj = o.n_obj;
        B.dynamic = s->model->dynamic_objects && s->T.obj_inertial != nullptr;
        HIP_OK(kp::launch_uhc_assign_obj(B, s->stream));
        o.on = true;
    } else
        HIP_OK(kp::launch_uhc_assign(A, s->stream));
    return launch_step(s, nullptr, 0, mask, false);
}

int kp_sim_step_head(kp_sim* s, const float* act) {
    if (!s || !act) return fail("kp_sim_step_head: null argument");
    HIP_OK(hipSetDevice(s->device));
    launch_target_fk(s, s->n, s->st.qpos, nullptr, s->tgt, kp::KinStep{act, s->st.xpos, s->st.xquat, s->st.prev_bquat, s->st.prev_hpos, 1.0f / 30.0f});
    return launched();
}

int kp_sim_step_kin(kp_sim* s, const float* act, float* next_qpos) {
    if (!s || !act || !next_qpos) return fail("kp_sim_step_kin: null argument");
    HIP_OK(hipSetDevice(s->device));
    hipLaunchKernelGGL(kp::k_step_kin, dim3((s->n + 63) / 64), dim3(64), 0, s->stream, s->n, s->st.qpos, act, next_qpos, 1.0f / 30.0f);
    return launched();
}

static kp::ObsCcArgs obs_cc_args(const kp_sim* s, float* out, const float* zf_mean, const float* zf_std, float clip) {
    kp::ObsCcArgs A;
    A.n = s->n; A.qpos = s->st.qpos; A.qvel = s->st.qvel; A.xpos = s->st.xpos; A.xquat = s->st.xquat; A.xipos = s->st.xipos;
    A.t_qpos = s->tgt.qpos; A.t_wbpos = s->tgt.wbpos; A.t_wbquat = s->tgt.wbquat; A.t_com = s->tgt.com;
    for (int k = 0; k < 4; k++) A.br_inv[k] = s->P.br_inv[k];
    A.zf_mean = zf_mean; A.zf_std = zf_std; A.clip = clip; A.out = out;
    return A;
}

extern "C++" {
using ObsCcLaunch = void (*)(kp_sim*, const kp::ObsCcArgs&, const float*);
template <int V, int I>
static void launch_obs_cc(kp_sim* s, const kp::ObsCcArgs& A, const float* phase) {
    if constexpr (V == 1 && I == 0) hipLaunchKernelGGL(kp::k_obs_cc_uhc, dim3(s->n), dim3(64), 0, s->stream, A);
    else hipLaunchKernelGGL((kp::k_obs_cc<V, (I & 1) != 0, (I & 2) != 0, (I & 4) != 0, (I & 8) != 0>), dim3(s->n), dim3(64), 0, s->stream, A, phase);
}
template <int... I>
static constexpr std::array<ObsCcLaunch, 20> obs_cc_table(std::integer_sequence<int, I...>) {
    return {launch_obs_cc<0, I>..., launch_obs_cc<1, 0>, launch_obs_cc<1, 1>, launch_obs_cc<2, 0>, launch_obs_cc<2, 1>};
}
static constexpr auto OBS_CC = obs_cc_table(std::make_integer_sequence<int, 16>{});
static constexpr int OBS_CC_V1 = 16;
}

int kp_sim_obs_cc(kp_sim* s, float* out, const float* zf_mean, const float* zf_std, float clip) {
    if (!s || !out) return fail("kp_sim_obs_cc: null argument");
    if ((zf_mean == nullptr) != (zf_std == nullptr)) return fail("kp_sim_obs_cc: pass both zf_mean and zf_std or neither");
    HIP_OK(hipSetDevice(s->device));
    OBS_CC[OBS_CC_V1](s, obs_cc_args(s, out, zf_mean, zf_std, clip), nullptr);
    return launched();
}

int kp_sim_obs_cc_ex(kp_sim* s, float* out, const float* zf_mean, const float* zf_std, float clip, const float* phase) {
    if (!s || !out) return fail("kp_sim_obs_cc_ex: null argument");
    if ((zf_mean == nullptr) != (zf_std == nullptr)) return fail("kp_sim_obs_cc_ex: pass both zf_mean and zf_std or neither");
    if (s->cc_obs_phase && !phase) return fail("kp_sim_obs_cc_ex: this handle's observation ends with the phase (cc_obs_phase = 1): pass phase [N]");
    if (!s->cc_obs_phase && phase) return fail("kp_sim_obs_cc_ex: phase given, but this handle's observation has no phase slot (cc_obs_phase = 0 or cc_obs_v != 0)");
    HIP_OK(hipSetDevice(s->device));
    const int i = s->cc_obs_v == 0 ? s->cc_obs_vel_root | s->cc_obs_heading << 1 | s->cc_obs_deheading << 2 | s->cc_obs_phase << 3
                                   : OBS_CC_V1 + 2 * (s->cc_obs_v - 1) + s->cc_obs_vel_root;
    OBS_CC[i](s, obs_cc_args(s, out, zf_mean, zf_std, clip), phase);
    return launched();
}
int kp_sim_cc_obs_dim(const kp_sim* s) { return s ? s->cc_obs_dim : -1; }

struct Field { int dim; bool view; float* (*row)(const kp_sim&); };
#define ROW(member) [](const kp_sim& s) -> float* { return s.member; }
static const Field FIELDS[] = {
     {76, true, ROW(st.qpos)},  {75, true, ROW(st.qvel)},  {72, true, ROW(st.xpos)},  {96, true, ROW(st.xquat)},
     {72, true, ROW(st.xipos)},  {96, false, nullptr},  {7, false, nullptr},
     {76, true, ROW(tgt.qpos)},  {72, false, ROW(tgt.wbpos)},  {96, false, ROW(tgt.wbquat)},
     {96, false, ROW(tgt.bquat)},  {72, false, ROW(tgt.com)},
     {76, true, ROW(st.qpos_d)},  {75, true, ROW(st.qvel_d)},
     {96, false, ROW(st.prev_bquat)},  {7, false, ROW(st.prev_hpos)},
     {35, true, ROW(obj.qpos)},  {30, true, ROW(obj.qvel)},  {75 * 75, false, nullptr},  {75, false, nullptr},
};
#undef ROW
static_assert(sizeof(FIELDS) / sizeof(FIELDS[0]) == KP_BIAS + 1, "one row per kp_field");
static const Field* find_field(int f) { return f >= 0 && f <= KP_BIAS ? &FIELDS[f] : nullptr; }

int kp_field_dim(int f) { const Field* d = find_field(f); return d ? d->dim : -1; }

__global__ void k_head(int n, const float* __restrict__ xpos, const float* __restrict__ xquat, float* __restrict__ out) {
    int e = blockIdx.x * blockDim.x + threadIdx.x;
    if (e >= n) return;
    const int hb = 13;
    for (int k = 0; k < 3; k++) out[(size_t)e * 7 + k] = xpos[(size_t)e * 72 + 3 * hb + k];
    for (int k = 0; k < 4; k++) out[(size_t)e * 7 + 3 + k] = xquat[(size_t)e * 96 + 4 * hb + k];
}

const float* kp_sim_field_device(kp_sim* s, int field) {
    const Field* d = find_field(field);
    return s && d && d->view ? d->row(*s) : nullptr;
}

int kp_sim_get(kp_sim* s, int field, float* out) {
    if (!s || !out) return fail("kp_sim_get: null argument");
    HIP_OK(hipSetDevice(s->device));
    const Field* d = find_field(field);
    if (!d) return fail("kp_sim_get: unknown field");
    if (d->row) {
        HIP_OK(hipMemcpyAsync(out, d->row(*s), sizeof(float) * (size_t)s->n * d->dim, hipMemcpyDeviceToDevice, s->stream));
        return 0;
    }
    if (field == KP_M) return kp_sim_mass_matrix(s, out, nullptr);
    if (field == KP_BIAS) return kp_sim_mass_matrix(s, nullptr, out);
    if (field == KP_BQUAT) hipLaunchKernelGGL(kp::k_bquat, dim3((s->n * 24 + 255) / 256), dim3(256), 0, s->stream, s->n, s->st.qpos, out);
    else hipLaunchKernelGGL(k_head, dim3((s->n + 255) / 256), dim3(256), 0, s->stream, s->n, s->st.xpos, s->st.xquat, out);
    return launched();
}

static kp::CtxDev to_dev(const kp_ctx* c) {
    kp::CtxDev d;
    d.T = c->T; d.head_pose = c->head_pose; d.head_vels = c->head_vels; d.obj_rel = c->obj_head_relative_poses;
    d.action_one_hot = c->action_one_hot; d.gt_bquat = c->gt_bquat; d.gt_wbpos = c->gt_wbpos; d.obj_qpos = c->obj_qpos; d.cur_t = c->cur_t; d.row = c->row;
    return d;
}

int kp_sim_step_begin(kp_sim* s) {
    if (!s) return fail("kp_sim_step_begin: null argument");
    HIP_OK(hipSetDevice(s->device));
    hipLaunchKernelGGL(kp::k_snapshot, dim3((s->n * 24 + 255) / 256), dim3(256), 0, s->stream, s->n, s->st.qpos, s->st.xpos, s->st.xquat, s->st.prev_bquat, s->st.prev_hpos);
    return launched();
}

extern "C++" {
template <int I>
static void launch_obs_ar(kp_sim* s, const kp_ctx* c, float* out) {
    constexpr bool VEL = (I & 1) != 0, HEAD = (I & 2) != 0, ACTION = (I & 4) != 0;
    static_assert(kp::ObsArLayout<VEL, HEAD, ACTION>::D == 74 + 75 * VEL + 7 * HEAD + 7 + 13 * HEAD + 4 * ACTION, "ar_obs_width is the kernel's row width");
    if constexpr (!VEL && HEAD)
        hipLaunchKernelGGL(kp::k_obs_ar_thread<ACTION>, dim3((s->n + 63) / 64), dim3(64), 0, s->stream, s->n, to_dev(c), s->st.qpos, s->st.xpos, s->st.xquat, out);
    else
        hipLaunchKernelGGL((kp::k_obs_ar<VEL, HEAD, ACTION>), dim3((s->n + 7) / 8), dim3(256), 0, s->stream, s->n, to_dev(c), s->st.qpos, s->st.qvel, s->st.xpos, s->st.xquat, out);
}
}
static void (*const OBS_AR[8])(kp_sim*, const kp_ctx*, float*) = {launch_obs_ar<0>, launch_obs_ar<1>, launch_obs_ar<2>, launch_obs_ar<3>,
                                                                  launch_obs_ar<4>, launch_obs_ar<5>, launch_obs_ar<6>, launch_obs_ar<7>};

static int check_obs_ar_args(const char* who, const kp_sim* s, const kp_ctx* c, const float* out) {
    if (!s || !c || !out || !c->head_pose || !c->head_vels || !c->obj_head_relative_poses || !c->action_one_hot || !c->cur_t || c->T < 1)
        return fail(std::string(who) + ": bad arguments");
    return 0;
}

int kp_sim_obs_ar(kp_sim* s, const kp_ctx* c, float* out) {
    if (check_obs_ar_args("kp_sim_obs_ar", s, c, out)) return -1;
    HIP_OK(hipSetDevice(s->device));
    OBS_AR[s->ar_obs_vel | s->ar_obs_head << 1 | s->ar_obs_action << 2](s, c, out);
    return launched();
}

static kp::RewardW reward_w(const kp_reward_cfg* w) {
    return kp::RewardW{w->w_hp, w->w_hq, w->w_p, w->w_jp, w->w_act_p, w->w_act_v, w->k_hp, w->k_hq, w->k_p, w->k_jp, w->k_act_p, w->k_act_v,
                       w->dt, w->body_diff_thresh, w->body_diff_gt_thresh, w->use_gt_term};
}
static int launch_term_reward(kp_sim* s, const kp_ctx* c, const kp_reward_cfg* w, float* reward, float* info, uint8_t* failp, float* diffs, const kp::PostStep* post) {
    const StateRows& st = s->st;
    if (!post) hipLaunchKernelGGL(kp::k_term_reward<false>, dim3((s->n + 7) / 8), dim3(256), 0, s->stream, s->n, to_dev(c), reward_w(w), st.qpos, st.xpos, st.xquat,
                                  s->tgt.wbpos, s->tgt.bquat, st.prev_bquat, st.prev_hpos, s->diffw, reward, info, failp, diffs, kp::PostStep{});
    else hipLaunchKernelGGL(kp::k_term_reward<true>, dim3((s->n + 7) / 8), dim3(256), 0, s->stream, s->n, to_dev(c), reward_w(w), st.qpos, st.xpos, st.xquat,
                            s->tgt.wbpos, s->tgt.bquat, st.prev_bquat, st.prev_hpos, s->diffw, reward, info, failp, diffs, *post);
    return launched();
}

int kp_sim_term_reward(kp_sim* s, const kp_ctx* c, const kp_reward_cfg* w, float* reward, float* info, uint8_t* failp, float* diffs) {
    if (!s || !c || !w || !reward || !info || !failp || !diffs || !c->head_pose || !c->gt_bquat || !c->gt_wbpos || !c->cur_t || c->T < 2)
        return fail("kp_sim_term_reward: bad arguments");
    HIP_OK(hipSetDevice(s->device));
    return launch_term_reward(s, c, w, reward, info, failp, diffs, nullptr);
}

int kp_sim_post_step(kp_sim* s, const kp_ctx* c, const kp_reward_cfg* w, int32_t* cur_t, const int32_t* row_len, int env_episode_len,
                     float* reward, float* info, uint8_t* failp, float* diffs, uint8_t* done, uint8_t* end, float* percent, int32_t* done_count, float* obj7) {
    if (!s || !c || !w || !cur_t || !row_len || !reward || !info || !failp || !diffs || !done || !end || !percent || !c->head_pose || !c->gt_bquat || !c->gt_wbpos || c->T < 2)
        return fail("kp_sim_post_step: bad arguments");
    if (c->cur_t != cur_t) return fail("kp_sim_post_step: cur_t must be the buffer the context reads (kp_ctx.cur_t)");
    if (obj7 && !c->action_one_hot) return fail("kp_sim_post_step: obj7 needs the context's action_one_hot");
    HIP_OK(hipSetDevice(s->device));
    const kp::PostStep PS{cur_t, row_len, env_episode_len, done, end, percent, done_count, obj7, obj7 ? s->obj.qpos : nullptr};
    return launch_term_reward(s, c, w, reward, info, failp, diffs, &PS);
}

static int launch_term_reward_v2(kp_sim* s, const kp_ctx* c, const kp_reward_cfg_v2* w, float* reward, float* info, uint8_t* failp, float* diffs, const kp::PostStep* post) {
    const StateRows& st = s->st;
    const kp::RewardW2 W{w->w_hp, w->w_hq, w->w_p, w->w_v, w->w_e, w->k_hp, w->k_hq, w->k_p, w->k_v, w->k_e, w->dt, w->body_diff_thresh, w->body_diff_gt_thresh,
                         w->use_gt_term, w->b_diffw};
    if (!post) hipLaunchKernelGGL((kp::k_term_reward<false, 2, kp::RewardW2>), dim3((s->n + 7) / 8), dim3(256), 0, s->stream, s->n, to_dev(c), W, st.qpos, st.xpos, st.xquat,
                                  s->tgt.wbpos, s->tgt.bquat, st.prev_bquat, st.prev_hpos, s->diffw, reward, info, failp, diffs, kp::PostStep{});
    else hipLaunchKernelGGL((kp::k_term_reward<true, 2, kp::RewardW2>), dim3((s->n + 7) / 8), dim3(256), 0, s->stream, s->n, to_dev(c), W, st.qpos, st.xpos, st.xquat,
                            s->tgt.wbpos, s->tgt.bquat, st.prev_bquat, st.prev_hpos, s->diffw, reward, info, failp, diffs, *post);
    return launched();
}

int kp_sim_term_reward_v2(kp_sim* s, const kp_ctx* c, const kp_reward_cfg_v2* w, float* reward, float* info, uint8_t* failp, float* diffs) {
    if (!s || !c || !w || !w->b_diffw || !reward || !info || !failp || !diffs || !c->head_pose || !c->gt_bquat || !c->gt_wbpos || !c->cur_t || c->T < 2)
        return fail("kp_sim_term_reward_v2: bad arguments");
    HIP_OK(hipSetDevice(s->device));
    return launch_term_reward_v2(s, c, w, reward, info, failp, diffs, nullptr);
}

int kp_sim_post_step_v2(kp_sim* s, const kp_ctx* c, const kp_reward_cfg_v2* w, int32_t* cur_t, const int32_t* row_len, int env_episode_len,
                        float* reward, float* info, uint8_t* failp, float* diffs, uint8_t* done, uint8_t* end, float* percent, int32_t* done_count, float* obj7) {
    if (!s || !c || !w || !w->b_diffw || !cur_t || !row_len || !reward || !info || !failp || !diffs || !done || !end || !percent || !c->head_pose || !c->gt_bquat ||
        !c->gt_wbpos || c->T < 2)
        return fail("kp_sim_post_step_v2: bad arguments");
    if (c->cur_t != cur_t) return fail("kp_sim_post_step_v2: cur_t must be the buffer the context reads (kp_ctx.cur_t)");
    if (obj7 && !c->action_one_hot) return fail("kp_sim_post_step_v2: obj7 needs the context's action_one_hot");
    HIP_OK(hipSetDevice(s->device));
    const kp::PostStep PS{cur_t, row_len, env_episode_len, done, end, percent, done_count, obj7, obj7 ? s->obj.qpos : nullptr};
    return launch_term_reward_v2(s, c, w, reward, info, failp, diffs, &PS);
}

int kp_sim_reset_rows(kp_sim* s, const float* init_qpos, const float* init_qvel, const int32_t* row, const uint8_t* mask, int32_t* cur_t, int set_target,
                      float* aux_rows, int aux_cols, const float* row_obj_qpos, const float* row_action_one_hot, float* obj7) {
    if (!s || !init_qpos || !init_qvel || (aux_rows && aux_cols <= 0)) return fail("kp_sim_reset_rows: null argument");
    if (obj7 && !row_obj_qpos) return fail("kp_sim_reset_rows: obj7 needs row_obj_qpos");
    HIP_OK(hipSetDevice(s->device));
    if (row_obj_qpos && launch_set_objects(s, "kp_sim_reset_rows", row_obj_qpos, mask, row, row_action_one_hot, obj7)) return -1;
    hipLaunchKernelGGL(kp::k_reset_rows, dim3(s->n), dim3(128), 0, s->stream, s->n, init_qpos, init_qvel, row, mask, cur_t, s->st.qpos, s->st.qvel, s->st.qpos_d, s->st.qvel_d,
                       s->st.warm, aux_rows, aux_rows ? aux_cols : 0);
    HIP_OK(hipGetLastError());
    if (int rc = launch_step(s, nullptr, 0, mask, false)) return rc;
    if (set_target) {
        launch_target_fk(s, s->n, s->st.qpos, mask, s->tgt);
        HIP_OK(hipGetLastError());
    }
    return 0;
}

int kp_gae_bootstrap(int n, int T, const float* rewards, const float* masks, const float* values, const float* last_values, float gamma, float tau,
                     float* adv, float* ret, void* stream) {
    if (n <= 0 || T <= 0 || !rewards || !masks || !values || !adv || !ret) return fail("kp_gae: bad arguments");
    hipLaunchKernelGGL(kp::k_gae, dim3((n + 63) / 64), dim3(64), 0, (hipStream_t)stream, n, T, rewards, masks, values, last_values, gamma, tau, adv, ret);
    return launched();
}
int kp_gae(int n, int T, const float* rewards, const float* masks, const float* values, float gamma, float tau, float* adv, float* ret, void* stream) {
    return kp_gae_bootstrap(n, T, rewards, masks, values, nullptr, gamma, tau, adv, ret, stream);
}

int kp_pool_advance(int n, int n_slots, const uint8_t* done, int32_t* head, int32_t* ahead, int32_t* row, void* stream) {
    if (n <= 0 || n_slots <= 0 || !done || !head || !ahead || !row) return fail("kp_pool_advance: bad arguments");
    hipLaunchKernelGGL(kp::k_pool_advance, dim3((n + 255) / 256), dim3(256), 0, (hipStream_t)stream, n, n_slots, done, head, ahead, row);
    return launched();
}

int kp_sim_ar_obs_dim(const kp_sim* s) { return s ? s->ar_obs_dim : -1; }

static int record_pre(const char* who, const kp_record_pre* r, int obs_dim, void* stream) {
    if ((r->states && !r->obs) || (r->episode_start && !r->fresh) || (r->curr_qpos && !r->qpos) || (r->meta && !r->row_meta) ||
        (r->gt_target_qpos && (!r->ctx_qpos || !r->cur_t || !r->row_len || r->ctx_T <= 0)))
        return fail(std::string(who) + ": a destination without its source");
    kp::RecordPre R{r->n, r->T, r->t, r->ctx_T, obs_dim, r->obs, r->fresh, r->qpos, r->ctx_qpos, r->row, r->cur_t, r->row_len, r->row_meta,
                    r->states, r->episode_start, r->curr_qpos, r->gt_target_qpos, r->meta};
    hipLaunchKernelGGL(kp::k_record_pre, dim3(r->n), dim3(128), 0, (hipStream_t)stream, R);
    return launched();
}
static int record_post(const char* who, const kp_record_post* r, int obs_dim, void* stream) {
    if ((r->actions && !r->action) || (r->rewards && !r->reward) || (r->fails && !r->fail) || (r->dones && !r->done) || (r->percents && !r->percent) ||
        (r->c_infos && !r->c_info) || (r->next_states && !r->obs) || (r->res_qpos && !r->qpos) || (r->cc_actions && !r->cc_action) ||
        (r->cc_states && !r->cc_state) || (r->v_metas && !r->meta))
        return fail(std::string(who) + ": a destination without its source");
    kp::RecordPost R{r->n, r->T, r->t, obs_dim, r->fr_num, r->action, r->reward, r->fail, r->done, r->percent, r->c_info, r->obs, r->qpos, r->cc_action, r->cc_state, r->meta,
                     r->actions, r->rewards, r->fails, r->dones, r->percents, r->c_infos, r->next_states, r->res_qpos, r->cc_actions, r->cc_states, r->v_metas};
    hipLaunchKernelGGL(kp::k_record_post, dim3(r->n), dim3(128), 0, (hipStream_t)stream, R);
    return launched();
}

int kp_rollout_record_pre_w(const kp_record_pre* r, int obs_dim, void* stream) {
    if (!r || r->n <= 0 || r->T <= 0 || r->t < 0 || r->t >= r->T) return fail("kp_rollout_record_pre: bad arguments");
    if (!ar_obs_width_known(obs_dim)) return fail("kp_rollout_record_pre: obs_dim must be " KP_AR_OBS_WIDTHS ", got " + std::to_string(obs_dim));
    return record_pre("kp_rollout_record_pre", r, obs_dim, stream);
}
int kp_rollout_record_pre(const kp_record_pre* r, void* stream) { return kp_rollout_record_pre_w(r, KP_AR_OBS_DIM, stream); }

int kp_rollout_record_post_w(const kp_record_post* r, int obs_dim, void* stream) {
    if (!r || r->n <= 0 || r->T <= 0 || r->t < 0 || r->t >= r->T) return fail("kp_rollout_record_post: bad arguments");
    if (!ar_obs_width_known(obs_dim)) return fail("kp_rollout_record_post: obs_dim must be " KP_AR_OBS_WIDTHS ", got " + std::to_string(obs_dim));
    return record_post("kp_rollout_record_post", r, obs_dim, stream);
}
int kp_rollout_record_post(const kp_record_post* r, void* stream) { return kp_rollout_record_post_w(r, KP_AR_OBS_DIM, stream); }

int kp_mcp_compose(int n, int K, int A, const float* logits, const float* prim, const float* noise, int noise_stride, const float* stdv, float* out, void* stream) {
    if (n <= 0 || K <= 0 || K > 64 || A <= 0 || !logits || !prim || !out || (noise && !stdv)) return fail("kp_mcp_compose: bad arguments");
    if (noise && noise_stride < A) return fail("kp_mcp_compose: noise_stride " + std::to_string(noise_stride) + " is smaller than the row width A = " + std::to_string(A));
    const size_t tot = (size_t)n * A;
    hipLaunchKernelGGL(kp::k_mcp_compose, dim3((unsigned)((tot + 255) / 256)), dim3(256), 0, (hipStream_t)stream, n, K, A, logits, prim, noise, noise_stride, stdv, out);
    return launched();
}

int kp_kin_advance(int n, const float* qpos, const float* kin_action, float dt, float* next_qpos, float* qvel_fd, void* stream) {
    if (n <= 0 || !qpos || !kin_action || !next_qpos || !qvel_fd || !(dt > 0.f)) return fail("kp_kin_advance: bad arguments");
    hipLaunchKernelGGL(kp::k_kin_advance, dim3((n + 127) / 128), dim3(128), 0, (hipStream_t)stream, n, qpos, kin_action, dt, next_qpos, qvel_fd);
    return launched();
}

int kp_mcp_tail(int n, int K, int J, int A, const float* h2, const float* b2, const float* w3, int ldw, const float* b3, const float* logits, const float* noise,
                int noise_stride, const float* stdv, float* out, void* stream) {
    if (n <= 0 || K <= 0 || K > 16 || J <= 0 || J % kp::MCP_CHUNK || A <= 0 || A > 80 || ldw < A || !h2 || !b2 || !w3 || !b3 || !logits || !out || (noise && !stdv))
        return fail("kp_mcp_tail: bad arguments (K <= 16 primitives, hidden width a multiple of 64, A <= 80 actions, ldw >= A)");
    const dim3 grid((unsigned)((n + 15) / 16)), block(64 * kp::MCP_WAVES);
    hipStream_t st = (hipStream_t)stream;
// ... 573 lines not shown
```

### kinpoly_amd/csrc/kp_step_kernel.hpp

```cpp
#pragma once
#include <type_traits>

#include "kp_step_device.hpp"

namespace kp {

struct PhaseClock {
    unsigned long long pc[8] = {0, 0, 0, 0, 0, 0, 0, 0}, t0 = 0, tstart = 0;
    __device__ __forceinline__ void lap(int i) { const unsigned long long t1 = __builtin_readcyclecounter(); pc[i] += t1 - t0; t0 = t1; }
};
template <bool Q, typename V> __device__ __forceinline__ V gld(const V* p) {
    if constexpr (Q) return __hip_atomic_load(const_cast<V*>(p), __ATOMIC_RELAXED, __HIP_MEMORY_SCOPE_AGENT);
    else return *p;
}
template <bool Q, typename V> __device__ __forceinline__ void gst(V* p, V v) {
    if constexpr (Q) __hip_atomic_store(p, v, __ATOMIC_RELAXED, __HIP_MEMORY_SCOPE_AGENT);
    else *p = v;
}

template <int NT, bool OBJ, bool FWD, bool Q = false, bool LEAN = false, bool XC = false, bool PROF = false>
__device__ __forceinline__ int step_body(const int env_in, const int part, const XcArgs* X = nullptr) {
    static_assert(!LEAN || (Q && !OBJ && !FWD && NT == 64), "the lean layout serves the floor scenes' job queue only");
    static_assert(!PROF || (!Q && !FWD), "the phase profiler runs on the one-workgroup-per-env step kernels");
    const StepArgs& A = kp_kernarg();
// ... 235 lines not shown
                                if (Q && A.warm_extrap != 0.f && A.obj_warm2 && part >= 0 && part + 1 < A.n_parts) gst<Q>(A.obj_warm2 + (size_t)envS * 6 * D_MAXOBJ + (unsigned)(6 * k + tidS), s.oqa_prev[6 * k + tidS]); }
            }
        }
    }
    if (bad) atomicOr(&s.flag, 1);
    KP_SYNC();
    if (tidS == 0 && A.diag && n_substeps > 0) {
        int* dg = A.diag + 4 * (size_t)envS;
        if (part > 0) {
            const int d3 = gld<Q>(dg + 3), d2 = gld<Q>(dg + 2);
            niter_total += gld<Q>(dg + 1); s.flag |= d2 & 255; ncap_total += d2 >> 8;
            maxcon = max(maxcon, d3 & 255); nfact_total += d3 >> 8;
        }
        gst<Q>(dg + 0, s.ncon); gst<Q>(dg + 1, niter_total); gst<Q>(dg + 2, (s.flag & 255) | (ncap_total << 8)); gst<Q>(dg + 3, maxcon | (nfact_total << 8));
    }
    if (tidS == 0 && A.cost && n_substeps > 0)
        gst<Q>(A.cost + envS, (part > 0 ? gld<Q>(A.cost + envS) : 0u) + (unsigned)((__builtin_readcyclecounter() - t_launch) >> 10));
    return 0;
}

__global__ __launch_bounds__(64) void kp_mass_kernel(StepArgs A, float* __restrict__ Mout, float* __restrict__ bias_out) {
    extern __shared__ __attribute__((aligned(16))) unsigned char smem_raw[];
    EnvLds& s = *reinterpret_cast<EnvLds*>(smem_raw);
    constexpr int NT = 64;
    const int tid = threadIdx.x, env = blockIdx.x;
    if (env >= A.n_envs) return;
    const DevTables& T = A.T;
    const Params& P = A.P;
    const int depth = tid < D_NB ? T.body_depth[tid] : -1;
    const V3 bpos = tid < D_NB ? ld3(T.body_pos + 3 * tid) : v3(0.f, 0.f, 0.f);
    for (int i = tid; i < D_NQ; i += NT) s.qpos[i] = A.qpos_d[(size_t)env * D_NQ + i];
    for (int i = tid; i < D_NV; i += NT) { s.qvel[i] = A.qvel_d[(size_t)env * D_NV + i]; s.arm[i] = T.dof_armature[i]; s.dbody[i] = T.dof_body[i]; }
    if (tid < D_NB) { s.bpar[tid] = (unsigned char)(T.body_parent[tid] < 0 ? 0 : T.body_parent[tid]); s.bsub[tid] = T.body_subtree[tid]; s.bdep[tid] = T.body_depth[tid]; }
    KP_SYNC();
    forward_kin_bias<NT>(s, T, P, depth, bpos, tid);
    for (int it = tid; it < D_NB * 6; it += NT) {
        const int b = it / 6, c = it - 6 * b, n = s.bsub[b];
        float acc = 0.f;
        for (int k = b; k < b + n; k++) acc += s.fb[6 * k + c];
        s.sa[it] = acc;
    }
    KP_SYNC();
    if (bias_out) for (int d = tid; d < D_NV; d += NT) bias_out[(size_t)env * D_NV + d] = dot6(lds6(s.cdof + 6 * d), lds6(s.sa + 6 * s.dbody[d]));
    KP_SYNC();
    if (!Mout) return;
    for (int j = 0; j < D_NV; j++) {
        for (int i = tid; i < D_NV; i += NT) s.x[i] = i == j ? 1.f : 0.f;
        KP_SYNC();
        spatial_accumulate<NT>(s, s.x, depth, tid);
        wrench_project<NT, false>(s, P, s.sv, s.x, nullptr, s.qacc_s, true, false, tid, s.arm);
        for (int d = tid; d < D_NV; d += NT) Mout[((size_t)env * D_NV + d) * D_NV + j] = s.qacc_s[d];
        KP_SYNC();
    }
}

__global__ __launch_bounds__(1024) void k_lpt_order(int n, const unsigned* __restrict__ cost, int* __restrict__ order) {
    __shared__ unsigned hist[256], base[256], cmax;
    const int tid = threadIdx.x;
    if (tid < 256) hist[tid] = 0;
    if (tid == 0) cmax = 1;
    __syncthreads();
    unsigned m = 0;
    for (int i = tid; i < n; i += 1024) m = max(m, cost[i]);
    atomicMax(&cmax, m);
    __syncthreads();
    const float sc = 255.f / (float)cmax;
    for (int i = tid; i < n; i += 1024) atomicAdd(&hist[255 - (int)((float)cost[i] * sc)], 1u);
    __syncthreads();
    if (tid == 0) { unsigned a = 0; for (int b = 0; b < 256; b++) { base[b] = a; a += hist[b]; } }
    __syncthreads();
    for (int i = tid; i < n; i += 1024) order[atomicAdd(&base[255 - (int)((float)cost[i] * sc)], 1u)] = i;
}

template <int NT, bool OBJ, bool PROF = false>
__global__ __launch_bounds__(NT, (NT == 64 ? 2 : 1)) void kp_step_kernel(StepArgs A) {
    step_body<NT, OBJ, false, false, false, false, PROF>(A.order ? A.order[blockIdx.x] : (int)blockIdx.x, -1);
}
template <int NT, bool OBJ, bool PROF = false>
__global__ __launch_bounds__(NT, (NT == 64 ? 2 : 1)) void kp_step_kernel_xc(StepArgs A, XcArgs X) {
    step_body<NT, OBJ, false, false, false, true, PROF>(A.order ? A.order[blockIdx.x] : (int)blockIdx.x, -1, &X);
}
template <int NT, bool OBJ>
__global__ __launch_bounds__(NT, (NT == 64 ? 2 : 1)) void kp_forward_kernel(StepArgs A) { step_body<NT, OBJ, true>((int)blockIdx.x, -1); }

template <bool OBJ, bool LEAN, bool XC>
__device__ __forceinline__ void step_queue_body(const StepArgs& A, const XcArgs* X) {
    const unsigned total = (unsigned)A.n_envs * (unsigned)A.n_parts;
    const unsigned prev_tot = A.jobctr[48], prev_cnt = A.jobctr[49];
    for (;;) {
        unsigned idx = 0;
        if (threadIdx.x == 0) idx = atomicAdd(&A.jobctr[0], 1u);
        idx = (unsigned)__builtin_amdgcn_readfirstlane((int)idx);
        if (idx >= total) return;
        unsigned e, spins = 0;
        unsigned long long t_wait = 0;
        while ((e = __hip_atomic_load(&A.jobq[idx], __ATOMIC_RELAXED, __HIP_MEMORY_SCOPE_AGENT)) == 0xFFFFFFFFu) {
            if (spins < 16u) __builtin_amdgcn_s_sleep(32);
            else for (unsigned k = 0; k <= min((spins - 16u) >> 3, 7u); k++) __builtin_amdgcn_s_sleep(127);
            if (idx >= total - __hip_atomic_load(&A.jobctr[16], __ATOMIC_RELAXED, __HIP_MEMORY_SCOPE_AGENT)) return;
            if (++spins == 1u) t_wait = __builtin_amdgcn_s_memrealtime();
            else if ((spins & 63u) == 0u && __builtin_amdgcn_s_memrealtime() - t_wait > 200000000ull) { if (threadIdx.x == 0) atomicExch(&A.jobctr[2], 1u); return; }
        }
        asm volatile("" ::: "memory");
        if (A.queue_fence) __builtin_amdgcn_fence(__ATOMIC_ACQUIRE, "agent");
        e = (unsigned)__builtin_amdgcn_readfirstlane((int)e);
        const int env = (int)(e & 0xFFFFFFu);
        int part = (int)(e >> 24);
        const bool late = A.queue_late && part == 0 && idx >= gridDim.x;
        if (A.queue_prio == 1) { if (A.order_valid && part == 0 && idx < (unsigned)A.n_envs / 16u) __builtin_amdgcn_s_setprio(2); else __builtin_amdgcn_s_setprio(0); }
        if (A.queue_prio == 2) { if (part == 0) __builtin_amdgcn_s_setprio(2); else if (part + 1 < A.n_parts) __builtin_amdgcn_s_setprio(1); else __builtin_amdgcn_s_setprio(0); }
        for (;;) {
            const unsigned long long tj = __builtin_amdgcn_s_memrealtime();
            const int overflow = step_body<64, OBJ, false, true, LEAN, XC>(env, part, X);
            asm volatile("s_waitcnt vmcnt(0) lgkmcnt(0)" ::: "memory");
            if (A.queue_fence) __builtin_amdgcn_fence(__ATOMIC_RELEASE, "agent");
            if (LEAN && overflow) {
                if (threadIdx.x == 0) {
                    A.ovfq[atomicAdd(&A.jobctr[64], 1u)] = (unsigned)env | ((unsigned)part << 24);
                    atomicAdd(&A.jobctr[16], (unsigned)(A.n_parts - 1 - part));
                }
                break;
            }
            if (part + 1 >= A.n_parts) break;
            int keep = 0;
            if (A.queue_heavy > 0 && threadIdx.x == 0) {
                const unsigned nsub = (unsigned)(((part < 8 ? A.part_sub_lo >> (8 * part) : A.part_sub_hi >> (8 * (part - 8)))) & 255ull);
                const unsigned dt = (unsigned)((__builtin_amdgcn_s_memrealtime() - tj) >> 2);
                atomicAdd(&A.jobctr[32], dt); atomicAdd(&A.jobctr[33], nsub);
                keep = prev_cnt >= 512u && nsub >= 4u && (unsigned long long)dt * prev_cnt * 100ull > (unsigned long long)prev_tot * nsub * (unsigned)A.queue_heavy;
            }
            keep = __builtin_amdgcn_readfirstlane(keep) | (int)late;
            if (!keep) {
                if (threadIdx.x == 0) {
                    const unsigned pos = atomicAdd(&A.jobctr[1], 1u);
                    __hip_atomic_store(&A.jobq[pos], (unsigned)env | ((unsigned)(part + 1) << 24), __ATOMIC_RELAXED, __HIP_MEMORY_SCOPE_AGENT);
                }
                break;
            }
            if (threadIdx.x == 0) atomicAdd(&A.jobctr[16], 1u);
            if (A.queue_prio == 1) __builtin_amdgcn_s_setprio(3);
            part++;
            if (A.queue_prio == 2) { if (part + 1 < A.n_parts) __builtin_amdgcn_s_setprio(2); else __builtin_amdgcn_s_setprio(1); }
        }
    }
}

template <bool OBJ, bool LEAN = false>
__global__ __launch_bounds__(64, (LEAN ? 3 : 2)) void kp_step_queue_kernel(StepArgs A) { step_queue_body<OBJ, LEAN, false>(A, nullptr); }
template <bool OBJ>
__global__ __launch_bounds__(64, 2) void kp_step_queue_kernel_xc(StepArgs A, XcArgs X) { step_queue_body<OBJ, false, true>(A, &X); }

__global__ __launch_bounds__(64, 2) void kp_step_overflow_kernel(StepArgs A) {
    for (;;) {
        unsigned idx = 0;
        if (threadIdx.x == 0) idx = atomicAdd(&A.jobctr[65], 1u);
        idx = (unsigned)__builtin_amdgcn_readfirstlane((int)idx);
        if (idx >= __hip_atomic_load(&A.jobctr[64], __ATOMIC_RELAXED, __HIP_MEMORY_SCOPE_AGENT)) return;
        const unsigned e = (unsigned)__builtin_amdgcn_readfirstlane((int)__hip_atomic_load(&A.ovfq[idx], __ATOMIC_RELAXED, __HIP_MEMORY_SCOPE_AGENT));
        const int env = (int)(e & 0xFFFFFFu);
        for (int part = (int)(e >> 24); part < A.n_parts; part++) {
            step_body<64, false, false, true, false>(env, part);
            asm volatile("s_waitcnt vmcnt(0) lgkmcnt(0)" ::: "memory");
            if (A.queue_fence) { __builtin_amdgcn_fence(__ATOMIC_RELEASE, "agent"); __builtin_amdgcn_fence(__ATOMIC_ACQUIRE, "agent"); }
        }
    }
}
// ... 9 lines not shown
```

### kinpoly_amd/env.py

```python
from __future__ import annotations

import numpy as np
import torch

from . import sim as kpsim
from .model_compiler import read_kpm
from .nets import PolicyMCP

CTX_KEYS = ("qpos", "head_pose", "head_vels", "obj_head_relative_poses", "action_one_hot", "init_qpos", "init_qvel")


class RunningState:

    def __init__(self, mean, std, clip=5.0, device="cuda"):
        self.mean = torch.as_tensor(mean, dtype=torch.float32, device=device).contiguous()
        self.std = torch.as_tensor(std, dtype=torch.float32, device=device).contiguous()
        self.clip = float(clip)

    @classmethod
    def identity(cls, dim=784, clip=5.0, device="cuda"):
        return cls(np.zeros(dim), np.ones(dim), clip, device)


class BatchedHumanoidAREnv:
# ... 227 lines not shown
            sub = {}
            for k, v in ctx.items():
                if k in ("len", "take_ind", "fr_start") and not torch.is_tensor(v):
                    v = torch.as_tensor(v)
                sub[k] = v.to(self.device)[idx] if torch.is_tensor(v) and v.dim() > 0 and v.shape[0] == R else v
            self.write_context_rows(idx, sub)

    def load_uhc_checkpoint(self, path, load_policy=True):
        from . import checkpoint as ck
        from .uhc_config import ConfigError
        cp = ck.load_checkpoint(path)
        arr = ck.running_state_arrays(cp.get("running_state"))
        if arr is not None and len(arr[0]) != kpsim.CC_OBS_DIM:
            raise ConfigError(f"{path}: running_state is {len(arr[0])}-d, a UHC of another obs_v / obs_vel; this env runs uhc.yml's controller "
                              f"(obs_v 1, obs_vel full: {kpsim.CC_OBS_DIM})")
        if load_policy and not any(k.startswith("composer.") for k in cp["policy_dict"]):
            raise ConfigError(f"{path}: policy_dict is not a PolicyMCP (actor_type gauss?); this env runs uhc.yml's controller (actor_type mcp)")
        ls = cp["policy_dict"].get("action_log_std")
        if load_policy and ls is not None and tuple(ls.shape)[-1] != kpsim.CC_ACTION_DIM:
            raise ConfigError(f"{path}: the policy's action is {tuple(ls.shape)[-1]}-d, a UHC with meta_pd / meta_pd_joint or residual_force off; this env runs "
                              f"uhc.yml's controller ({kpsim.CC_ACTION_DIM})")
        if arr is not None:
            self.cc_running_state = RunningState(arr[0], arr[1], arr[2], self.device)
        if load_policy:
            self.cc_policy.load_state_dict({k: (v if torch.is_tensor(v) else torch.as_tensor(v)) for k, v in cp["policy_dict"].items()})
            self.cc_policy.to(self.device).float()
        return cp

    @property
    def has_objects(self):
        return self._row_obj_qpos is not None

    @property
    def obj_qpos(self):
        return self.sim.get("obj_qpos") if self.has_objects else None

    def render_rgb(self, envs=None, camera=None, width=320, height=240):
        from .render import render_env
        return render_env(self.sim, self.obj_qpos, envs, camera, width, height)

    def render_ego(self, envs=None, width=64, height=64, camera=None):
        from .render import render_env_ego
        return render_env_ego(self.sim, self.obj_qpos, envs, camera, width, height)

    @property
    def ctx_len(self):
        return self.row_len[self.row.long()]

    def set_rows(self, new_row: torch.Tensor, env_mask: torch.Tensor | None = None):
        nr = new_row.to(self.device, torch.int32)
        if env_mask is None:
            self.row.copy_(nr)
        else:
            self.row.copy_(torch.where(env_mask.to(self.device, torch.bool), nr, self.row))

    def ctx_rows(self, key):
        return self.ctx[key][self.row.long()]

    @staticmethod
    def _mask8(env_mask, device):
        if env_mask is None:
            return None
        m = env_mask.to(device)
        return (m.view(torch.uint8) if m.dtype == torch.bool else m.to(torch.uint8)).contiguous()

    def reset(self, env_mask: torch.Tensor | None = None, policy_state: torch.Tensor | None = None):
        m8 = self._mask8(env_mask, self.device)
        self.sim.reset_rows(self._init_q, self._init_v, self.row, m8, self.cur_t, set_target=True, aux_rows=policy_state,
                            row_obj_qpos=self._row_obj_qpos, row_one_hot=None if self._row_obj_qpos is None else self.ctx["action_one_hot"], obj7=self.obj7)
        return self._obs_ar(self._obs)

    def _ar_frame(self, key):
        t = (self.cur_t.long() + 1).clamp_(max=self.ctx[key].shape[1] - 1)
        return self.ctx[key][self.row.long(), t].contiguous()

    def ar_fail_safe(self, env_mask: torch.Tensor | None = None):
        self.sim.set_state(self._ar_frame("ar_qpos"), self._ar_frame("ar_qvel"), self._mask8(env_mask, self.device))

    def step(self, a: torch.Tensor, need_obs: bool = True, cc_noise: torch.Tensor | None = None):
        sim = self.sim
        if self.ar_mode:
            sim.step_begin()
            sim.set_target(self._ar_frame("ar_qpos"))
        else:
            sim.step_head(a)
        rs = self.cc_running_state
        cc_obs = sim.obs_cc(self._cc_obs, rs.mean, rs.std, rs.clip)
        mean_action = self.mode == "test" or (self.mode == "train" and self.joint_controller)
        with torch.no_grad():
            cc_action = self.cc_policy.select_action(cc_obs, mean_action, self.gen, cc_noise).contiguous()
        sim.step_ctrl(cc_action, self.frame_skip)
        self._last_cc_action = cc_action
        self._flip ^= 1
        o = self._outs[self._flip]
        sim.post_step(self._ctx_struct, self.reward_cfg, self.cur_t, self.row_len, int(min(self.env_episode_len, 2 ** 31 - 1)),
                      o["reward"], o["info"], o["fail"], o["diffs"], o["done"], o["end"], o["percent"], self.done_count, self.obj7)
        if self.push_schedule is not None:
            bad = (~torch.isfinite(o["diffs"]).all(1)).to(torch.uint8)
            o["fail"] |= bad; o["done"] |= bad
            entity, impulse, offset = self.push_schedule.draw(self.cur_t, o["done"] == 0)
            sim.apply_impulse(entity, impulse, offset)
        obs = self._obs_ar(self._obs_next) if need_obs else None
        info = {"fail": o["fail"].view(torch.bool), "end": o["end"].view(torch.bool), "percent": o["percent"], "cc_action": cc_action, "cc_state": cc_obs,
                "custom_reward": o["reward"], "custom_info": o["info"], "body_diff": o["diffs"]}
        return obs, self._unit_reward, o["done"].view(torch.bool), info

    def push(self, entity, impulse, offset=None, env_mask=None):
        self.sim.apply_impulse(entity.to(self.device, torch.int32).contiguous(), impulse.to(self.device, torch.float32).contiguous(),
                               None if offset is None else offset.to(self.device, torch.float32).contiguous(), self._mask8(env_mask, self.device))

    def contact_forces(self, cc_action=None, **kw) -> dict:
        if "torque" in kw:
            if cc_action is not None:
                raise ValueError("contact_forces: cc_action and torque are mutually exclusive")
            return self.sim.contact_forces(**kw)
        if cc_action is None:
            cc_action = getattr(self, "_last_cc_action", None)
            if cc_action is None:
                raise RuntimeError("contact_forces(): no cc_action yet -- call step() first, or pass cc_action")
        return self.sim.contact_forces(action=cc_action.to(self.device, torch.float32).contiguous(), **kw)

    def body_motion(self, qacc=None, outputs=("body_vel", "body_com_vel", "centroid")) -> dict:
        return self.sim.body_motion(self.sim.view("qpos"), self.sim.view("qvel"), qacc, outputs=outputs)

    def centroidal(self, qacc=None) -> dict:
        from . import balance
        return balance.centroidal(self.sim, self.sim.view("qpos"), self.sim.view("qvel"), qacc)

    def get_humanoid_qpos(self):
        return self.sim.get("qpos")

    def get_humanoid_qvel(self):
        return self.sim.get("qvel")

    def get_head(self):
        return self.sim.get("head")

    def get_body_quat(self):
        return self.sim.get("bquat")

    def get_wbody_pos(self):
        return self.sim.get("xpos")

    def get_wbody_quat(self):
        return self.sim.get("xquat")

    def get_body_com(self):
        return self.sim.get("xipos")

    @property
    def target(self):
        g = self.sim.get
        return {"qpos": g("target_qpos"), "wbpos": g("target_wbpos"), "wbquat": g("target_wbquat"), "bquat": g("target_bquat"),
                "body_com": g("target_com")}


ACTION_INDEX_MAP, ACTION_LEN = (0, 7, 21, 28), (7, 14, 7, 7)


def convert_obj_qpos(action_one_hot: torch.Tensor, obj_pose0: torch.Tensor):
    n, dev = action_one_hot.shape[0], action_one_hot.device
    blk = torch.zeros((n, 35), device=dev)
    for i in range(5):
        blk[:, 7 * i] = (i + 1) * 100.0; blk[:, 7 * i + 1] = 100.0
    obj7 = torch.tensor([0.0, 0, 0, 1, 0, 0, 0], device=dev).repeat(n, 1)
    for a in range(4):
        m = (action_one_hot[:, a] > 0).unsqueeze(1)
        st, ln = ACTION_INDEX_MAP[a], min(ACTION_LEN[a], obj_pose0.shape[1])
        blk[:, st:st + ln] = torch.where(m, obj_pose0[:, :ln], blk[:, st:st + ln])
        obj7 = torch.where(m, blk[:, st:st + 7], obj7)
# ... 184 lines not shown
```

### kinpoly_amd/sim.py

```python
from __future__ import annotations

import ctypes as C
import os

import numpy as np
import torch

from . import build as _build

NQ, NV, NU, NBODY = 76, 75, 69, 24
CC_OBS_DIM, AR_OBS_DIM, KIN_ACTION_DIM, CC_ACTION_DIM = 784, 105, 80, 75
AR_OBS_DIM_NO_ACTION = 101


def ar_obs_dim(use_vel=False, use_head=True, use_action=True) -> int:
    return 74 + 75 * bool(use_vel) + 7 * bool(use_head) + 7 + 13 * bool(use_head) + 4 * bool(use_action)


AR_OBS_DIMS = tuple(ar_obs_dim(v, h, a) for h in (True, False) for v in (False, True) for a in (True, False))


def ar_obs_options(use_vel=False, use_head=True, use_action=True) -> dict:
    return {k: int(v) for k, v, d in (("ar_obs_vel", use_vel, False), ("ar_obs_head", use_head, True), ("ar_obs_action", use_action, True)) if bool(v) != d}
DEFAULT_KPM = os.path.join(os.path.dirname(os.path.abspath(__file__)), "assets", "smpl_humanoid.kpm")
# ... 123 lines not shown


FIT_INFO = {"cost0": 0, "cost": 1, "accepted": 2, "mu": 3, "max_epos": 4, "max_erot": 5, "dq_inf": 6, "status": 7}


class KpMarkerSet(C.Structure):
    _fields_ = [("n_points", C.c_int), ("pt_body", C.c_void_p), ("pt_offset", C.c_void_p)]


class KpFitPointsIn(C.Structure):
    _fields_ = [(k, C.c_void_p) for k in ("qpos0", "pt_tgt", "pt_w", "tgt_pos", "tgt_quat", "w_pos", "w_rot", "q_prior", "w_prior")]


class KpFitPointsCfg(C.Structure):
    _fields_ = [("fit", KpFitCfg), ("w_floor", C.c_float), ("floor_z", C.c_float)]

    @classmethod
    def default(cls):
        c = cls()
        load_library().kp_fit_points_cfg_default(C.byref(c))
        return c


class KpFitPointsOut(C.Structure):
    _fields_ = [(k, C.c_void_p) for k in ("qpos", "info", "dq", "pt_err")]


FIT_POINTS_INFO = {**FIT_INFO, "max_ept": 8, "rms_ept": 9, "max_depth": 10, "n_below": 11}
MAX_POINTS = 1024


class KpEstimateCfg(C.Structure):
    _fields_ = [(k, C.c_float) for k in ("reach", "w_f", "w_m", "rho", "mu")] + [("n_iters", C.c_int)]

    @classmethod
    def default(cls, model):
        c = cls()
        load_library().kp_estimate_cfg_default(model.h, C.byref(c))
        return c


class KpEstimateOut(C.Structure):
    _fields_ = [(k, C.c_void_p) for k in ("qfrc_inverse", "qfrc_contact", "contact", "lambda", "resid", "net_wrench", "ncon", "info")]


ESTIMATE_OUTPUTS = {"qfrc_inverse": ((75,), torch.float32), "qfrc_contact": ((75,), torch.float32), "contact": ((64, 12), torch.float32),
                    "lambda": ((64, 4), torch.float32), "resid": ((6,), torch.float32), "net_wrench": ((6,), torch.float32), "ncon": ((), torch.int32),
                    "info": ((8,), torch.float32)}
ESTIMATE_INFO = {"cost0": 0, "cost": 1, "iters": 2, "active": 3, "f_norm": 4, "searches": 5, "reserved": 6, "status": 7}


class KinPolyNativeError(RuntimeError):
    pass


_V, _I, _F, _D, _S = C.c_void_p, C.c_int, C.c_float, C.c_double, C.c_char_p
_PI = C.POINTER(C.c_int)
_CTX, _RW, _PRE, _POST, _UST, _UCFG, _EXT, _STYLE = (C.POINTER(k) for k in (KpCtx, KpRewardCfg, KpRecordPre, KpRecordPost, KpUhcState, KpUhcCfg, KpObsExt, KpRenderStyle))
_SIGNATURES = {
    "kp_last_error": (_S, []), "kp_version": (_S, []),
    "kp_model_load": (_V, [_S]), "kp_model_compile": (_I, [_S, _S, _S]), "kp_model_load_xml": (_V, [_S, _S]), "kp_model_free": (None, [_V]),
    "kp_model_set_option": (_I, [_V, _S, _D]), "kp_model_get_option": (_D, [_V, _S]),
    "kp_sim_create": (_V, [_V, _I, _I, _V]), "kp_sim_destroy": (None, [_V]), "kp_sim_n_envs": (_I, [_V]), "kp_sim_set_stream": (_I, [_V, _V]),
    "kp_sim_status_device": (_V, [_V]), "kp_sim_contacts": (_I, [_V, _V]), "kp_sim_mass_matrix": (_I, [_V, _V, _V]),
    "kp_sim_set_state": (_I, [_V, _V, _V, _V]), "kp_sim_set_full_state": (_I, [_V, _V, _V, _V, _V, _V]), "kp_sim_set_target": (_I, [_V, _V, _V]),
    "kp_sim_set_objects": (_I, [_V, _V, _V]), "kp_sim_set_obj_state": (_I, [_V, _V, _V, _V]),
    "kp_sim_apply_impulse": (_I, [_V, _V, _V, _V, _V, _V]),
    "kp_sim_contact_forces": (_I, [_V, _I, _V, _V, _V]),
    "kp_sim_inverse_dynamics": (_I, [_V, _I, _V, _V, _V, _V, _V]),
    "kp_sim_body_motion": (_I, [_V, _I, _V, _V, _V, _V]),
    "kp_sim_point_jacobian": (_I, [_V, _I, _V, _V, _V, _V]),
    "kp_fit_cfg_default": (None, [C.POINTER(KpFitCfg)]),
    "kp_sim_fit_pose": (_I, [_V, _I, _V, _V, _V]),
    "kp_fit_points_cfg_default": (None, [C.POINTER(KpFitPointsCfg)]),
    "kp_sim_fit_points": (_I, [_V, _I, _V, _V, _V, _V]),
    "kp_estimate_cfg_default": (None, [_V, C.POINTER(KpEstimateCfg)]),
    "kp_sim_estimate_contacts": (_I, [_V, _I, _V, _V, _V, _V, _V, _V]),
    "kp_sim_fk": (_I, [_V, _I, _V, _V, _V, _V, _V, _V]), "kp_sim_fk_backward": (_I, [_V, _I, _V, _V, _V, _V, _V]),
    "kp_sim_pose_contacts": (_I, [_V, _I, _V, _V, _V, _F, _V, _V, _V]),
    "kp_model_hull_planes": (_I, [_V, _V, _V]), "kp_render_style_default": (None, [_STYLE]),
    "kp_sim_render": (_I, [_V, _I, _I, _V, _V, _V, _V, _I, _I, _I, _STYLE, _V, _V, _V]),
    "kp_sim_render_ego": (_I, [_V, _I, _I, _V, _V, _V, _V, _V, _V, _V, _V, _I, _I, _I, _I, _STYLE, _I, _I, _V, _V, _V, _V, _V, _V]),
    "kp_sim_step_ctrl": (_I, [_V, _V, _I, _V]), "kp_sim_step_ctrl_base": (_I, [_V, _V, _I, _V, _V]), "kp_sim_step_kin": (_I, [_V, _V, _V]),
    "kp_sim_step_head": (_I, [_V, _V]), "kp_sim_step_begin": (_I, [_V]),
    "kp_sim_obs_cc": (_I, [_V, _V, _V, _V, _F]), "kp_sim_obs_cc_ex": (_I, [_V, _V, _V, _V, _F, _V]), "kp_sim_cc_obs_dim": (_I, [_V]),
    "kp_sim_obs_ar": (_I, [_V, _CTX, _V]), "kp_sim_ar_obs_dim": (_I, [_V]),
    "kp_field_dim": (_I, [_I]), "kp_sim_get": (_I, [_V, _I, _V]), "kp_sim_field_device": (_V, [_V, _I]),
    "kp_sim_term_reward": (_I, [_V, _CTX, _RW, _V, _V, _V, _V]),
    "kp_sim_post_step": (_I, [_V, _CTX, _RW, _V, _V, _I, _V, _V, _V, _V, _V, _V, _V, _V, _V]),
    "kp_sim_term_reward_v2": (_I, [_V, _CTX, C.POINTER(KpRewardCfgV2), _V, _V, _V, _V]),
    "kp_sim_post_step_v2": (_I, [_V, _CTX, C.POINTER(KpRewardCfgV2), _V, _V, _I, _V, _V, _V, _V, _V, _V, _V, _V, _V]),
    "kp_sim_reset_rows": (_I,[_V, _V, _V, _V, _V, _V, _I, _V, _I, _V, _V, _V]),
    "kp_sim_diag": (_I, [_V, _V]), "kp_sim_lean_state": (_I, [_V, _V]), "kp_sim_launch_cost": (_I, [_V, _V]), "kp_job_schedule": (_I, [_I, _I, _I, _PI]),
    "kp_sim_last_step_seconds": (_D, [_V]), "kp_sim_timing_reset": (_I, [_V]), "kp_sim_timing_mean_seconds": (_D, [_V, _PI]),
    "kp_sim_phase_cycles": (_I, [_V, C.POINTER(_D)]), "kp_sim_phase_cycles_env": (_I, [_V, _V]),
    "kp_takes_create": (_V, [_V, _V, _I, _V, _I, _D]), "kp_takes_destroy": (None, [_V]),
    "kp_takes_create_obj": (_V, [_V, _V, _V, _I, _V, _I, _D]), "kp_takes_has_objects": (_I, [_V]),
    "kp_takes_table": (_I, [_V, _S, C.POINTER(_V), _PI, _PI]), "kp_takes_info": (_I, [_V, _PI, _PI, _V]),
    "kp_sim_uhc_track": (_I, [_V, _V, _UST, _UCFG, _V, _V, _V, _V, _V, _V, _V, _V]), "kp_sim_uhc_assign": (_I, [_V, _V, _UST, _UCFG, _V, _V, _V, _I, _V]),
    "kp_uhc_reward_info_dim": (_I, [_I]), "kp_sim_uhc_track_r": (_I, [_V, _V, _UST, C.POINTER(KpUhcCfgR), _V, _V, _V, _V, _V, _V, _V, _V]),
    "kp_pool_advance": (_I, [_I, _I, _V, _V, _V, _V, _V]),
    "kp_rollout_record_pre": (_I, [_PRE, _V]), "kp_rollout_record_post": (_I, [_POST, _V]),
    "kp_rollout_record_pre_w": (_I, [_PRE, _I, _V]), "kp_rollout_record_post_w": (_I, [_POST, _I, _V]),
    "kp_mcp_compose": (_I, [_I, _I, _I, _V, _V, _V, _I, _V, _V, _V]),
    "kp_mcp_tail": (_I, [_I, _I, _I, _I, _V, _V, _V, _I, _V, _V, _V, _I, _V, _V, _V]),
    "kp_kin_advance": (_I, [_I, _V, _V, _F, _V, _V, _V]), "kp_gru_cell_step": (_I, [_I, _I, _I, _V, _V, _V, _V, _V, _V, _V, _V, _V]),
    "kp_gae": (_I, [_I, _I, _V, _V, _V, _F, _F, _V, _V, _V]), "kp_gae_bootstrap": (_I, [_I, _I, _V, _V, _V, _V, _F, _F, _V, _V, _V]),
    "kp_gru_gates_forward": (_I, [_I, _I, _V, _V, _V, _V, _V, _V, _V]), "kp_gru_gates_backward": (_I, [_I, _I, _V, _V, _V, _V, _V, _V, _V, _V, _V, _V]),
    "kp_kin_advance_backward": (_I, [_I, _V, _V, _F, _V, _V, _V, _V, _V]),
    "kp_sim_obs_ar_backward": (_I, [_V, _CTX, _I, _I, _V, _V, _V, _V, _V, _V, _V, _V, _V]),
    "kp_sim_fk_head_backward": (_I, [_V, _I, _V, _V, _V, _V, _V, _V, _V, _V]),
    "kp_sim_obs_ar_ex": (_I, [_V, _CTX, _EXT, _V]),
    "kp_sim_obs_ar_ex_backward": (_I, [_V, _CTX, _EXT, _I, _I, _V, _V, _V, _V, _V, _V, _V, _V, _V, _V]),
    "kp_rollout_record_pre_x": (_I, [_PRE, _I, _I, _I, _V]), "kp_rollout_record_post_x": (_I, [_POST, _I, _I, _I, _V]),
    "kp_ctx_rows_write": (_I, [_I, _I, _I, _I, _I, _I, _V, _V, _V, _V, _V, _V, _V]),
}
ABI_SYMBOLS = list(_SIGNATURES)


def load_library(path: str | None = None):
    global _lib
    if _lib is not None:
        return _lib
    path = path or os.environ.get("KP_SIM_LIBRARY") or _build.LIB
    if not os.path.exists(path):
        raise KinPolyNativeError(f"{path} is missing: run `python -c 'import __graft_entry__ as g; g.build()'` "
                                 "(hipcc --offload-arch=gfx950). There is no CPU fallback.")
    L = C.CDLL(path)
    for sym, (restype, argtypes) in _SIGNATURES.items():
        f = getattr(L, sym)
        f.restype, f.argtypes = restype, argtypes
    _lib = L
    return L


def _check(rc, what):
    if rc != 0:
        raise KinPolyNativeError(f"{what}: {load_library().kp_last_error().decode()}")


def compile_model_native(xml_path: str, uhc_yml: str | None, out_kpm: str):
    L = load_library()
    _check(L.kp_model_compile(xml_path.encode(), None if uhc_yml is None else uhc_yml.encode(), out_kpm.encode()), "kp_model_compile")


class KpModel:
    def __init__(self, kpm_path: str = DEFAULT_KPM, xml: tuple | None = None, **options):
        self.L = load_library()
        self.kpm_path = None if xml is not None else kpm_path
        if xml is not None:
            self.h = self.L.kp_model_load_xml(xml[0].encode(), None if xml[1] is None else xml[1].encode())
        else:
            self.h = self.L.kp_model_load(kpm_path.encode())
        if not self.h:
            raise KinPolyNativeError(f"kp_model_load: {self.L.kp_last_error().decode()}")
        for k, v in options.items():
            self.set_option(k, v)

    def hull_planes(self):
        n = self.L.kp_model_hull_planes(self.h, None, None)
        if n < 0:
            raise KinPolyNativeError(f"kp_model_hull_planes: {self.L.kp_last_error().decode()}")
        planes, adr = np.empty((n, 4), np.float32), np.empty(NBODY + 1, np.int32)
        self.L.kp_model_hull_planes(self.h, planes.ctypes.data_as(C.c_void_p), adr.ctypes.data_as(C.c_void_p))
        return planes, adr

    def set_option(self, name, value):
# ... 133 lines not shown
            self._stream = stream

    def status_tensor(self) -> torch.Tensor:
        if getattr(self, "_status", None) is None:
            self._status = _device_view(self.L.kp_sim_status_device(self.h), (4,), self.device, "<i4")
        return self._status

    def queue_counters(self) -> dict:
        if getattr(self, "_qctr", None) is None:
            self._qctr = _device_view(self.L.kp_sim_status_device(self.h), (128,), self.device, "<i4")
        c = self._qctr.cpu().numpy()
        st = (C.c_int32 * 3)()
        _check(self.L.kp_sim_lean_state(self.h, C.cast(st, C.c_void_p)), "kp_sim_lean_state")
        return {"claimed": int(c[0]), "published": int(c[1]), "stalled": int(c[2]), "kept_by_their_wave": int(c[16]), "lean_overflow_jobs": int(c[64]),
                "lean_layout_next_launch": bool(st[0]), "fallbacks_to_full_layout": int(st[1]), "control_step_launches": int(st[2])}

    def record_contacts(self):
        _check(self.L.kp_sim_contacts(self.h, None), "kp_sim_contacts")

    def contacts(self):
        buf = np.zeros((self.n, 1 + 64 * 9), np.float32)
        _check(self.L.kp_sim_contacts(self.h, buf.ctypes.data_as(C.c_void_p)), "kp_sim_contacts")
        out = []
        for e in range(self.n):
            n = int(buf[e, 0]); r = buf[e, 1:1 + 9 * n].reshape(n, 9).astype(np.float64)
            out.append(dict(body=r[:, 0].astype(int), b2=r[:, 1].astype(int), dist=r[:, 2], pos=r[:, 3:6], normal=r[:, 6:9]))
        return out

    def mass_matrix(self):
        M = torch.empty((self.n, 75, 75), dtype=torch.float32, device=self.device); b = self._new(75)
        _check(self.L.kp_sim_mass_matrix(self.h, C.c_void_p(M.data_ptr()), C.c_void_p(b.data_ptr())), "kp_sim_mass_matrix")
        return M, b

    def __del__(self):
        try:
            self.L.kp_sim_destroy(self.h)
        except Exception:
            pass

    def _new(self, dim):
        return torch.empty((self.n, dim), dtype=torch.float32, device=self.device)

    def set_state(self, qpos, qvel, env_mask=None):
        _check(self.L.kp_sim_set_state(self.h, _ptr(qpos, self.n, NQ), _ptr(qvel, self.n, NV), _mask_ptr(env_mask, self.n)), "kp_sim_set_state")

    def set_objects(self, obj_qpos, env_mask=None):
        _check(self.L.kp_sim_set_objects(self.h, _ptr(obj_qpos, self.n, 35), _mask_ptr(env_mask, self.n)), "kp_sim_set_objects")

    def set_obj_state(self, obj_qpos, obj_qvel, env_mask=None):
        _check(self.L.kp_sim_set_obj_state(self.h, _ptr(obj_qpos, self.n, 35), _ptr(obj_qvel, self.n, 30), _mask_ptr(env_mask, self.n)), "kp_sim_set_obj_state")

    def set_target(self, target_qpos, env_mask=None):
        _check(self.L.kp_sim_set_target(self.h, _ptr(target_qpos, self.n, NQ), _mask_ptr(env_mask, self.n)), "kp_sim_set_target")

    def step_ctrl(self, cc_action, n_substeps=15, env_mask=None):
        _check(self.L.kp_sim_step_ctrl(self.h, _ptr(cc_action, self.n, self.cc_action_dim), int(n_substeps), _mask_ptr(env_mask, self.n)), "kp_sim_step_ctrl")

    def step_ctrl_base(self, cc_action, base_qpos, n_substeps=15, env_mask=None):
        _check(self.L.kp_sim_step_ctrl_base(self.h, _ptr(cc_action, self.n, self.cc_action_dim), int(n_substeps), _mask_ptr(env_mask, self.n),
                                            _ptr(base_qpos, self.n, NQ)), "kp_sim_step_ctrl_base")

    def uhc_track(self, takes, st, cfg, cc_action, reward, info, body_diff, fail, end, done, percent):
        _check(self.L.kp_sim_uhc_track(self.h, takes.h, C.byref(st), C.byref(cfg), _ptr(cc_action, self.n, self.cc_action_dim), C.c_void_p(reward.data_ptr()),
                                       _ptr(info, self.n, 5), C.c_void_p(body_diff.data_ptr()), _mask_ptr(fail, self.n), _mask_ptr(end, self.n), _mask_ptr(done, self.n),
                                       C.c_void_p(percent.data_ptr())), "kp_sim_uhc_track")

    def uhc_track_r(self, takes, st, cfg, cc_action, reward, info, body_diff, fail, end, done, percent):
        _check(self.L.kp_sim_uhc_track_r(self.h, takes.h, C.byref(st), C.byref(cfg), _ptr(cc_action, self.n, self.cc_action_dim), C.c_void_p(reward.data_ptr()),
                                         _ptr(info, self.n, uhc_reward_info_dim(cfg.reward_id)), C.c_void_p(body_diff.data_ptr()), _mask_ptr(fail, self.n),
                                         _mask_ptr(end, self.n), _mask_ptr(done, self.n), C.c_void_p(percent.data_ptr())), "kp_sim_uhc_track_r")

    def uhc_assign(self, takes, st, cfg, env_mask=None, take_ids=None, start=None, keep_t=False, noise=None):
        ids = None if take_ids is None else np.ascontiguousarray(take_ids, np.int32)
        st0 = None if start is None else np.ascontiguousarray(start, np.int32)
        for a in (ids, st0):
            if a is not None and a.shape != (self.n,):
                raise ValueError(f"uhc_assign: take_ids / start must have shape ({self.n},)")
        _check(self.L.kp_sim_uhc_assign(self.h, takes.h, C.byref(st), C.byref(cfg), _mask_ptr(env_mask, self.n), None if ids is None else ids.ctypes.data_as(C.c_void_p),
                                        None if st0 is None else st0.ctypes.data_as(C.c_void_p), int(bool(keep_t)), _ptr(noise, self.n, NU)), "kp_sim_uhc_assign")

    def step_head(self, kin_action):
        _check(self.L.kp_sim_step_head(self.h, _ptr(kin_action, self.n, KIN_ACTION_DIM)), "kp_sim_step_head")

    def step_kin(self, kin_action, out=None):
        out = self._new(NQ) if out is None else out
        _check(self.L.kp_sim_step_kin(self.h, _ptr(kin_action, self.n, KIN_ACTION_DIM), _ptr(out, self.n, NQ)), "kp_sim_step_kin")
        return out

    def obs_cc(self, out=None, zf_mean=None, zf_std=None, clip=0.0, phase=None):
        out = self._new(self.cc_obs_dim) if out is None else out
        zm, zs = (_dev("ZFilter mean / std", z if z is None or not z.is_contiguous() else z.view(-1), (self.cc_obs_dim,)) for z in (zf_mean, zf_std))
        ph = None if phase is None else _ptr(phase.view(self.n, 1), self.n, 1)
        _check(self.L.kp_sim_obs_cc_ex(self.h, _ptr(out, self.n, self.cc_obs_dim), zm, zs, float(clip), ph), "kp_sim_obs_cc_ex")
        return out

    def get(self, field: str, out=None):
        fid = FIELDS[field]
        dim = self.L.kp_field_dim(fid)
        out = self._new(dim) if out is None else out
        _check(self.L.kp_sim_get(self.h, fid, _ptr(out, self.n, dim)), "kp_sim_get")
        return out

    def view(self, field: str) -> torch.Tensor:
        cache = self.__dict__.setdefault("_views", {})
        if field not in cache:
            fid = FIELDS[field]
            ptr = self.L.kp_sim_field_device(self.h, fid)
            if not ptr:
                raise KinPolyNativeError(f"kp_sim_field_device: '{field}' is not a stored field")
            cache[field] = _device_view(ptr, (self.n, self.L.kp_field_dim(fid)), self.device)
        return cache[field]

    def set_full_state(self, qpos, qvel, qpos_d, qvel_d, env_mask=None):
        _check(self.L.kp_sim_set_full_state(self.h, _ptr(qpos, self.n, NQ), _ptr(qvel, self.n, NV), _ptr(qpos_d, self.n, NQ),
                                            _ptr(qvel_d, self.n, NV), _mask_ptr(env_mask, self.n)), "kp_sim_set_full_state")

    def apply_impulse(self, entity, impulse, offset=None, env_mask=None, want_dqvel=False):
        dq = self._new(NV) if want_dqvel else None
        _check(self.L.kp_sim_apply_impulse(self.h, _dev("entity", entity, (self.n,), torch.int32), _dev("offset", offset, (self.n, 3)),
                                           _dev("impulse", impulse, (self.n, 6)), _mask_ptr(env_mask, self.n), _ptr(dq, self.n, NV)), "kp_sim_apply_impulse")
        return dq

    def contact_forces(self, action=None, torque=None, env_mask=None, want=tuple(CONTACT_OUTPUTS)) -> dict:
        if action is not None and torque is not None:
            raise ValueError("contact_forces: action and torque are mutually exclusive")
        want = _rows_want("contact_forces", want, CONTACT_OUTPUTS)
        mode, act = (2, _dev("action", action, (self.n, self.cc_action_dim))) if action is not None else (1, _dev("torque", torque, (self.n, NV))) if torque is not None else (0, None)
        out = _rows_outputs(self.n, CONTACT_OUTPUTS, want, self.device)
        _check(self.L.kp_sim_contact_forces(self.h, mode, act, _mask_ptr(env_mask, self.n), C.byref(_rows_struct(KpContactOut, CONTACT_OUTPUTS, out))), "kp_sim_contact_forces")
        return out

    def inverse_dynamics(self, qpos, qvel=None, qacc=None, obj_qpos=None, want=("qfrc_inverse",)) -> dict:
        want = _rows_want("inverse_dynamics", want, INVDYN_OUTPUTS)
        spec = _motion_spec(qpos, qvel, qacc, obj_qpos)
        lead, R, rows = _rows_inputs("inverse_dynamics", spec)
        ins = _rows_ptrs("inverse_dynamics", spec, rows)
        out = _rows_outputs(R, INVDYN_OUTPUTS, want, self.device)
        if R > 0:
            _check(self.L.kp_sim_inverse_dynamics(self.h, R, *ins, C.byref(_rows_struct(KpInvDynOut, INVDYN_OUTPUTS, out))), "kp_sim_inverse_dynamics")
        return _rows_view(out, lead)

    def estimate_contacts(self, qpos, qvel=None, qacc=None, obj_qpos=None, cfg: KpEstimateCfg | None = None, want=("qfrc_inverse",)) -> dict:
        want = _rows_want("estimate_contacts", want, ESTIMATE_OUTPUTS)
        spec = _motion_spec(qpos, qvel, qacc, obj_qpos)
        lead, R, rows = _rows_inputs("estimate_contacts", spec)
        ins = _rows_ptrs("estimate_contacts", spec, rows)
        cfg = KpEstimateCfg.default(self.model) if cfg is None else cfg
        out = _rows_outputs(R, ESTIMATE_OUTPUTS, want, self.device)
        if R > 0:
            _check(self.L.kp_sim_estimate_contacts(self.h, R, *ins, C.byref(cfg), C.byref(_rows_struct(KpEstimateOut, ESTIMATE_OUTPUTS, out))), "kp_sim_estimate_contacts")
        return _rows_view(out, lead)

    def body_motion(self, qpos, qvel=None, qacc=None, outputs=tuple(MOTION_OUTPUTS)) -> dict:
        want = _rows_want("body_motion", outputs, MOTION_OUTPUTS, "outputs")
        spec = _motion_spec(qpos, qvel, qacc)[:3]
        lead, R, rows = _rows_inputs("body_motion", spec)
        ins = _rows_ptrs("body_motion", spec, rows)
        out = _rows_outputs(R, MOTION_OUTPUTS, want, self.device)
        if R > 0:
            _check(self.L.kp_sim_body_motion(self.h, R, *ins, C.byref(_rows_struct(KpMotionOut, MOTION_OUTPUTS, out))), "kp_sim_body_motion")
        return _rows_view(out, lead)

    def point_jacobian(self, qpos, body, offset=None) -> torch.Tensor:
        spec = [("qpos", qpos, (NQ,), torch.float32, True), ("body", body, (), torch.int32, True), ("offset", offset, (3,), torch.float32, False)]
        lead, R, rows = _rows_inputs("point_jacobian", spec)
        ins = _rows_ptrs("point_jacobian", spec, rows)
# ... 551 lines not shown
```

Measured before the change: 1.417 million.

## Fuse head step with CC observation and compact reset rows into a list

Adds a fused kernel that runs the target forward kinematics for the head step and then builds the 784-wide CC observation in the same block, reading the target row from shared memory instead of global buffers. Reset handling now compacts masked envs into a device list, and the forward and target-FK kernels iterate only over that list. The grid is sized from a mapped host counter written by the previous reset. Both aim to cut launch count and idle blocks at episode boundaries. The cost is more LDS per block, a one-env-per-64-thread-block fused layout, and a reset grid sized from last call's count that relies on grid-stride loops for correctness.

```diff
diff --git a/include/kinpoly_sim.h b/include/kinpoly_sim.h
--- a/include/kinpoly_sim.h
+++ b/include/kinpoly_sim.h
@@ -70,6 +70,8 @@
 int kp_sim_step_head(kp_sim*, const float* kin_action);
 
 int kp_sim_obs_cc(kp_sim*, float* out, const float* zf_mean, const float* zf_std, float clip);
+
+int kp_sim_step_head_obs_cc(kp_sim*, const float* kin_action, float* out, const float* zf_mean, const float* zf_std, float clip);
 
 int kp_sim_obs_cc_ex(kp_sim*, float* out, const float* zf_mean, const float* zf_std, float clip, const float* phase);
 int kp_sim_cc_obs_dim(const kp_sim*);
diff --git a/kinpoly_amd/csrc/kp_obs_kernels.hpp b/kinpoly_amd/csrc/kp_obs_kernels.hpp
--- a/kinpoly_amd/csrc/kp_obs_kernels.hpp
+++ b/kinpoly_amd/csrc/kp_obs_kernels.hpp
@@ -60,14 +60,12 @@
 
 struct TargetBufs { float *qpos, *wbpos, *wbquat, *bquat, *com; };
 struct KinStep { const float *act, *xpos, *xquat; float *prev_bquat, *prev_hpos; float dt; };
-__global__ __launch_bounds__(256) void k_target_fk(int n, const float* __restrict__ tq, const uint8_t* __restrict__ mask, TargetBufs B,
+struct TargetRow { const float *qpos, *wbpos, *wbquat, *com; };
+template <int ROWS, bool HOLD = false>
+__device__ __forceinline__ TargetRow target_fk_body(const int w, const int lane, const int e, const bool live, const float* __restrict__ tq, const TargetBufs& B,
                                                     const float* __restrict__ body_pos, const float* __restrict__ body_ipos, const int8_t* __restrict__ parent,
-                                                    const uint8_t* __restrict__ depth, KinStep K = KinStep{nullptr, nullptr, nullptr, nullptr, nullptr, 0.f}) {
-    __shared__ float sq[4][80], swq[4][D_NB * 4], swp[4][D_NB * 3];
-    const int w = threadIdx.x >> 6, lane = threadIdx.x & 63;
-    const int e = blockIdx.x * 4 + w;
-    const bool live = e < n && !(mask && !mask[e]);
-    if (!__syncthreads_or(live)) return;
+                                                    const uint8_t* __restrict__ depth, const KinStep& K) {
+    __shared__ float sq[ROWS][80], swq[ROWS][D_NB * 4], swp[ROWS][D_NB * 3], scom[HOLD ? ROWS : 1][HOLD ? D_NB * 3 : 1];
     if (live) {
         const float* q = tq + (size_t)e * D_NQ;
         if (K.act) {
@@ -129,11 +127,41 @@
         if (B.bquat) { float* o = B.bquat + (size_t)e * 96 + 4 * b; o[0] = bq.w; o[1] = bq.x; o[2] = bq.y; o[3] = bq.z; }
         if (B.wbpos) st3(B.wbpos + (size_t)e * 72 + 3 * b, pos);
         if (B.wbquat) { float* o = B.wbquat + (size_t)e * 96 + 4 * b; o[0] = wqb.w; o[1] = wqb.x; o[2] = wqb.y; o[3] = wqb.z; }
-        if (B.com) st3(B.com + (size_t)e * 72 + 3 * b, q_mul_vec(wqb, ld3(body_ipos + 3 * b)) + pos);
+        if (B.com || HOLD) {
+            const V3 c = q_mul_vec(wqb, ld3(body_ipos + 3 * b)) + pos;
+            if (B.com) st3(B.com + (size_t)e * 72 + 3 * b, c);
+            if constexpr (HOLD) st3(scom[w] + 3 * b, c);
+        }
     }
     if (live && B.qpos) {
         float* oq = B.qpos + (size_t)e * D_NQ;
         for (int i = lane; i < D_NQ; i += 64) oq[i] = (i >= 3 && i < 7) ? swq[w][i - 3] : sq[w][i];
+    }
+    if constexpr (HOLD) {
+        __syncthreads();
+        if (live && lane < 4) sq[w][3 + lane] = swq[w][lane];
+        __syncthreads();
+    }
+    return TargetRow{sq[w], swp[w], swq[w], scom[w]};
+}
+__global__ __launch_bounds__(256) void k_target_fk(int n, const float* __restrict__ tq, const uint8_t* __restrict__ mask, TargetBufs B,
+                                                    const float* __restrict__ body_pos, const float* __restrict__ body_ipos, const int8_t* __restrict__ parent,
+                                                    const uint8_t* __restrict__ depth, KinStep K = KinStep{nullptr, nullptr, nullptr, nullptr, nullptr, 0.f}) {
+    const int w = threadIdx.x >> 6, lane = threadIdx.x & 63;
+    const int e = blockIdx.x * 4 + w;
+    const bool live = e < n && !(mask && !mask[e]);
+    if (!__syncthreads_or(live)) return;
+    target_fk_body<4>(w, lane, e, live, tq, B, body_pos, body_ipos, parent, depth, K);
+}
+__global__ __launch_bounds__(256) void k_target_fk_list(int n, const float* __restrict__ tq, const int* __restrict__ list, const unsigned* __restrict__ cnt, TargetBufs B,
+                                                         const float* __restrict__ body_pos, const float* __restrict__ body_ipos, const int8_t* __restrict__ parent,
+                                                         const uint8_t* __restrict__ depth) {
+    const int w = threadIdx.x >> 6, lane = threadIdx.x & 63;
+    const unsigned m = min(*cnt, (unsigned)n);
+    for (unsigned base = blockIdx.x * 4u; base < m; base += gridDim.x * 4u) {
+        const bool live = base + w < m;
+        const int e = live ? list[base + w] : 0;
+        target_fk_body<4>(w, lane, e, live && e >= 0 && e < n, tq, B, body_pos, body_ipos, parent, depth, KinStep{nullptr, nullptr, nullptr, nullptr, nullptr, 0.f});
     }
 }
 
@@ -206,7 +234,7 @@
     static constexpr int D = V == 0 ? (HEAD ? 1 : 0) + 74 + LV + 69 + (PHASE ? 1 : 0) : 229 + LV + (V == 1 ? 4 : 2) * 72 + 2 * 96;
 };
 template <int V, bool VROOT, bool HEAD, bool DEHEAD, bool PHASE>
-__device__ __forceinline__ void obs_cc_body(const ObsCcArgs& A, const float* __restrict__ phase) {
+__device__ __forceinline__ void obs_cc_body(const ObsCcArgs& A, const float* __restrict__ phase, const TargetRow* held = nullptr) {
     using L = ObsCcLayout<V, VROOT, HEAD, DEHEAD, PHASE>;
     constexpr int LV = L::LV, D = L::D;
     __shared__ float ob[D];
@@ -214,7 +242,11 @@
     if (e >= A.n) return;
     const float* qpos = A.qpos + (size_t)e * D_NQ;
     const float* qvel = A.qvel + (size_t)e * D_NV;
-    const float* tq = A.t_qpos + (size_t)e * D_NQ;
+    const float* tq = held ? held->qpos : A.t_qpos + (size_t)e * D_NQ;
+    const float* t_wbpos = held ? held->wbpos : A.t_wbpos + (size_t)e * 72;
+    const float* t_wbquat = held ? held->wbquat : A.t_wbquat + (size_t)e * 96;
+    const float* t_com = held ? held->com : A.t_com + (size_t)e * 72;
+    (void)t_wbpos; (void)t_wbquat; (void)t_com;
     const Q4 rq = Q4{qpos[3], qpos[4], qpos[5], qpos[6]};
     if constexpr (V == 0) {
         constexpr int H = HEAD ? 1 : 0, K = H + 74 + LV;
@@ -259,7 +291,7 @@
             const float* xi = A.xipos + (size_t)e * 72 + 3 * b;
             const float* xq = A.xquat + (size_t)e * 96;
             V3 cj = ld3(xp), ci = ld3(xi);
-            V3 tj = ld3(A.t_wbpos + (size_t)e * 72 + 3 * b), tc = ld3(A.t_com + (size_t)e * 72 + 3 * b);
+            V3 tj = ld3(t_wbpos + 3 * b), tc = ld3(t_com + 3 * b);
             V3 p1 = q_tmul_vec(crq, cj - root), p2 = q_tmul_vec(crq, tj - cj), p3 = q_tmul_vec(crq, ci - root), p4 = q_tmul_vec(crq, tc - ci);
             ob[P + b] = p1.x; ob[P + 24 + b] = p1.y; ob[P + 48 + b] = p1.z;
             ob[P + 72 + b] = p2.x; ob[P + 96 + b] = p2.y; ob[P + 120 + b] = p2.z;
@@ -267,7 +299,7 @@
                 ob[P + 144 + b] = p3.x; ob[P + 168 + b] = p3.y; ob[P + 192 + b] = p3.z;
                 ob[P + 216 + b] = p4.x; ob[P + 240 + b] = p4.y; ob[P + 264 + b] = p4.z;
             }
-            const float* twq = A.t_wbquat + (size_t)e * 96 + 4 * b;
+            const float* twq = t_wbquat + 4 * b;
             Q4 tqt = Q4{twq[0], twq[1], twq[2], twq[3]};
             Q4 cq = (xq[0] == 0.f) ? tqt : Q4{xq[4 * b], xq[4 * b + 1], xq[4 * b + 2], xq[4 * b + 3]};
             Q4 r1 = qmul(q_inverse(hq), cq), r2 = qmul(q_inverse(cq), tqt);
@@ -289,4 +321,13 @@
 __global__ __launch_bounds__(64) void k_obs_cc(ObsCcArgs A, const float* __restrict__ phase) { obs_cc_body<V, VROOT, HEAD, DEHEAD, PHASE>(A, phase); }
 __global__ __launch_bounds__(64) void k_obs_cc_uhc(ObsCcArgs A) { obs_cc_body<1, false, false, false, false>(A, nullptr); }
 
-}
+__global__ __launch_bounds__(64) void k_step_head_obs_cc_uhc(const float* __restrict__ tq, TargetBufs B, const float* __restrict__ body_pos,
+                                                              const float* __restrict__ body_ipos, const int8_t* __restrict__ parent,
+                                                              const uint8_t* __restrict__ depth, KinStep K, ObsCcArgs A) {
+    const int e = blockIdx.x;
+    if (e >= A.n) return;
+    const TargetRow R = target_fk_body<1, true>(0, threadIdx.x, e, true, tq, B, body_pos, body_ipos, parent, depth, K);
+    obs_cc_body<1, false, false, false, false>(A, nullptr, &R);
+}
+
+}
diff --git a/kinpoly_amd/csrc/kp_rollout_kernels.hpp b/kinpoly_amd/csrc/kp_rollout_kernels.hpp
--- a/kinpoly_amd/csrc/kp_rollout_kernels.hpp
+++ b/kinpoly_amd/csrc/kp_rollout_kernels.hpp
@@ -194,6 +194,35 @@
     if (i == 0 && cur_t) cur_t[e] = 0;
 }
 
+constexpr int RESET_SPAN = 16;
+__global__ __launch_bounds__(256) void k_reset_rows_list(int n, const float* __restrict__ init_qpos, const float* __restrict__ init_qvel, const int* __restrict__ row,
+                                                          const uint8_t* __restrict__ mask, int* __restrict__ cur_t, float* __restrict__ qpos, float* __restrict__ qvel,
+                                                          float* __restrict__ qpos_d, float* __restrict__ qvel_d, float* __restrict__ warm, float* __restrict__ aux_rows, int aux_cols,
+                                                          int* __restrict__ list, unsigned* __restrict__ cnt, unsigned* __restrict__ cnt_next) {
+    const int w = threadIdx.x >> 6, lane = threadIdx.x & 63;
+    if (blockIdx.x == 0 && threadIdx.x == 0) *cnt_next = 0u;
+    const int e0 = blockIdx.x * RESET_SPAN + lane;
+    const bool hit = lane < RESET_SPAN && e0 < n && mask[e0] != 0;
+    unsigned long long bits = __ballot(hit);
+    if (!bits) return;
+    if (w == 0) {
+        unsigned base = 0;
+        if (lane == 0) base = atomicAdd(cnt, (unsigned)__popcll(bits));
+        base = (unsigned)__builtin_amdgcn_readfirstlane((int)base);
+        const unsigned at = base + (unsigned)__popcll(bits & ((1ull << lane) - 1ull));
+        if (hit && at < (unsigned)n) list[at] = e0;
+    }
+    for (int k = 0; bits; k++, bits &= bits - 1ull) {
+        if ((k & 3) != w) continue;
+        const int e = blockIdx.x * RESET_SPAN + (__ffsll((long long)bits) - 1);
+        for (int c = lane; c < aux_cols; c += 64) aux_rows[(size_t)e * aux_cols + c] = 0.f;
+        const size_t r = row ? (size_t)row[e] : (size_t)e;
+        for (int i = lane; i < D_NQ; i += 64) { const float v = init_qpos[r * D_NQ + i]; qpos[(size_t)e * D_NQ + i] = v; qpos_d[(size_t)e * D_NQ + i] = v; }
+        for (int i = lane; i < D_NV; i += 64) { const float v = init_qvel[r * D_NV + i]; qvel[(size_t)e * D_NV + i] = v; qvel_d[(size_t)e * D_NV + i] = v; warm[(size_t)e * D_NV + i] = 0.f; }
+        if (lane == 0 && cur_t) cur_t[e] = 0;
+    }
+}
+
 __global__ void k_pool_advance(int n, int n_slots, const uint8_t* __restrict__ done, int* __restrict__ head, int* __restrict__ ahead, int* __restrict__ row) {
     const int e = blockIdx.x * blockDim.x + threadIdx.x;
     if (e >= n || !done[e]) return;
diff --git a/kinpoly_amd/csrc/kp_sim.hip b/kinpoly_amd/csrc/kp_sim.hip
--- a/kinpoly_amd/csrc/kp_sim.hip
+++ b/kinpoly_amd/csrc/kp_sim.hip
@@ -36,7 +36,7 @@
 
 struct kp_model {
     kp::HostModel h;
-    int contact = 1, limits = 1, stale = 1, solver_iter = 100, threads = 64, dynamic_objects = 1, lpt_order = -1, substeps_per_job = 4, queue_slots = 0, job_taper = 1, queue_fence = 1, queue_heavy = 160, queue_prio = -1, queue_late = -1, job_auto = 1, lean_queue = 1, lean_adaptive = 1, lds_pad = 0, lean_cap = kp::EnvLdsLean::MAXCON;
+    int contact = 1, limits = 1, stale = 1, solver_iter = 100, threads = 64, dynamic_objects = 1, lpt_order = -1, substeps_per_job = 4, queue_slots = 0, job_taper = 1, queue_fence = 1, queue_heavy = 160, queue_prio = -1, queue_late = -1, job_auto = 1, lean_queue = 1, lean_adaptive = 1, boundary_fused = 1, lds_pad = 0, lean_cap = kp::EnvLdsLean::MAXCON;
     double warm_extrap = -1.0;
     int planemesh_max = 3; double planemesh_tol = 0.3;
     int ar_obs_action = 1;
@@ -64,6 +64,11 @@
     long lean_off_until = -1; int fallbacks = 0;
     unsigned last = 0;
 };
+struct ResetList {
+    int* list = nullptr; unsigned* cnt = nullptr;
+    unsigned *host = nullptr, *host_dev = nullptr;
+    int turn = 0;
+};
 struct ObjectRows {
     float *qpos = nullptr, *geoms = nullptr;
     float *qvel = nullptr, *warm = nullptr, *warm2 = nullptr;
@@ -111,6 +116,7 @@
     kp::TargetBufs tgt{};
     JobQueue q;
     OverflowReadback ovf;
+    ResetList rl;
     ObjectRows obj;
     RenderTables rd;
     InvDynScratch idyn;
@@ -339,7 +345,11 @@
 }
 
 template <int NT, bool OBJ>
-void launch_per_env(const kp_sim* s, const kp::StepArgs& A, int nsub, size_t lds) {
+void launch_per_env(const kp_sim* s, const kp::StepArgs& A, int nsub, size_t lds, int list_grid) {
+    if (nsub == 0 && list_grid > 0) {
+        hipLaunchKernelGGL((kp::kp_forward_list_kernel<NT, OBJ>), dim3(list_grid), dim3(NT), lds, s->stream, A, s->rl.list, s->rl.cnt + s->rl.turn, s->rl.host_dev);
+        return;
+    }
     if (nsub > 0 && s->prof && s->xc_on) hipLaunchKernelGGL((kp::kp_step_kernel_xc<NT, OBJ, true>), dim3(s->n), dim3(NT), lds, s->stream, A, s->xc);
     else if (nsub > 0 && s->prof) hipLaunchKernelGGL((kp::kp_step_kernel<NT, OBJ, true>), dim3(s->n), dim3(NT), lds, s->stream, A);
     else if (nsub > 0 && s->xc_on) hipLaunchKernelGGL((kp::kp_step_kernel_xc<NT, OBJ>), dim3(s->n), dim3(NT), lds, s->stream, A, s->xc);
@@ -411,7 +421,7 @@
     return 0;
 }
 
-int launch_step(kp_sim* s, const float* action, int nsub, const uint8_t* mask, bool time_it, const float* base_qpos = nullptr) {
+int launch_step(kp_sim* s, const float* action, int nsub, const uint8_t* mask, bool time_it, const float* base_qpos = nullptr, int list_grid = 0) {
     const int threads = s->model->threads;
     if (s->obj.on && threads != 64) return fail("object contact needs threads_per_env = 64");
     if (threads != 64 && threads != 128 && threads != 256) return fail("threads_per_env must be 64, 128 or 256");
@@ -431,10 +441,10 @@
     kp::StepArgs A = step_args(s, p, nsub, action, mask, base_qpos);
     if (p.lpt) hipLaunchKernelGGL(kp::k_lpt_order, dim3(1), dim3(1024), 0, s->stream, s->n, s->q.cost, s->q.order);
     if (p.queue) { if (launch_queue(s, p, A, nsub, capturing)) return -1; }
-    else if (s->obj.on) launch_per_env<64, true>(s, A, nsub, p.lds);
-    else if (p.threads == 64) launch_per_env<64, false>(s, A, nsub, p.lds);
-    else if (p.threads == 128) launch_per_env<128, false>(s, A, nsub, p.lds);
-    else launch_per_env<256, false>(s, A, nsub, p.lds);
+    else if (s->obj.on) launch_per_env<64, true>(s, A, nsub, p.lds, list_grid);
+    else if (p.threads == 64) launch_per_env<64, false>(s, A, nsub, p.lds, list_grid);
+    else if (p.threads == 128) launch_per_env<128, false>(s, A, nsub, p.lds, list_grid);
+    else launch_per_env<256, false>(s, A, nsub, p.lds, list_grid);
     HIP_OK(hipGetLastError());
     return time_it ? timing_end(s, e0, e1) : 0;
 }
@@ -519,6 +529,7 @@
     OPT_I("queue_fence", O_BOOL, queue_fence), OPT_I("queue_heavy", O_CLAMP, queue_heavy, 0, INT_MAX),
     OPT_I("queue_late", O_TRI, queue_late), OPT_I("queue_prio", O_CLAMP, queue_prio, -1, 3),
     OPT_I("lean_queue", O_BOOL, lean_queue), OPT_I("lean_adaptive", O_BOOL, lean_adaptive),
+    OPT_I("boundary_fused", O_BOOL, boundary_fused),
     OPT_I("lean_max_contacts", O_RANGE, lean_cap, 0, kp::EnvLdsLean::MAXCON),
     OPT_I("lds_pad", O_RANGE, lds_pad, 0, 65536, "0 .. 65536 bytes"),
     OPT_RO("lds_bytes_per_env", (double)sizeof(kp::EnvLds)), OPT_RO("lds_bytes_per_env_objects", (double)sizeof(kp::EnvLdsObj)),
@@ -588,6 +599,14 @@
     q.order = (int*)dalloc(s, N, &ok); q.cost = (unsigned*)dalloc(s, N, &ok);
     q.jobq = (unsigned*)dalloc(s, N * 16, &ok); q.jobctr = (unsigned*)dalloc(s, 128, &ok); q.ovfq = (unsigned*)dalloc(s, N, &ok);
     q.spd_next = dalloc(s, N * 80, &ok);
+    ResetList& rl = s->rl;
+    rl.list = (int*)dalloc(s, N, &ok); rl.cnt = (unsigned*)dalloc(s, 2, &ok);
+    if (ok && hipMemset(rl.cnt, 0, 2 * sizeof(unsigned)) != hipSuccess) ok = false;
+    if (hipHostMalloc((void**)&rl.host, sizeof(unsigned), hipHostMallocMapped) != hipSuccess) rl.host = nullptr;
+    else {
+        *rl.host = (unsigned)n_envs;
+        if (hipHostGetDevicePointer((void**)&rl.host_dev, rl.host, 0) != hipSuccess) { hipHostFree(rl.host); rl.host = nullptr; rl.host_dev = nullptr; }
+    }
     hipDeviceProp_t prop;
     if (hipGetDeviceProperties(&prop, s->device) == hipSuccess && prop.multiProcessorCount > 0) q.wave_slots = prop.multiProcessorCount * 8;
     ObjectRows& o = s->obj;
@@ -621,6 +640,7 @@
     if (s->idyn.buf) hipFree(s->idyn.buf);
     if (s->mk.buf) hipFree(s->mk.buf);
     for (hipEvent_t e : s->tm.ring) hipEventDestroy(e);
+    if (s->rl.host) hipHostFree(s->rl.host);
     if (s->ovf.host) { hipHostFree(s->ovf.host); for (hipEvent_t e : s->ovf.ev) if (e) hipEventDestroy(e); }
     if (s->tm.ev0) hipEventDestroy(s->tm.ev0);
     if (s->tm.ev1) hipEventDestroy(s->tm.ev1);
@@ -1191,6 +1211,20 @@
 }
 int kp_sim_cc_obs_dim(const kp_sim* s) { return s ? s->cc_obs_dim : -1; }
 
+int kp_sim_step_head_obs_cc(kp_sim* s, const float* act, float* out, const float* zf_mean, const float* zf_std, float clip) {
+    if (!s || !act || !out) return fail("kp_sim_step_head_obs_cc: null argument");
+    if ((zf_mean == nullptr) != (zf_std == nullptr)) return fail("kp_sim_step_head_obs_cc: pass both zf_mean and zf_std or neither");
+    if (s->cc_obs_v != 1 || s->cc_obs_vel_root) return fail("kp_sim_step_head_obs_cc: the handle's observation is not get_full_obs_v1 with the full velocities (784 wide)");
+    if (!s->model->boundary_fused) {
+        if (int rc = kp_sim_step_head(s, act)) return rc;
+        return kp_sim_obs_cc(s, out, zf_mean, zf_std, clip);
+    }
+    HIP_OK(hipSetDevice(s->device));
+    hipLaunchKernelGGL(kp::k_step_head_obs_cc_uhc, dim3(s->n), dim3(64), 0, s->stream, s->st.qpos, s->tgt, s->T.body_pos, s->T.body_ipos, s->T.body_parent, s->T.body_depth,
+                       kp::KinStep{act, s->st.xpos, s->st.xquat, s->st.prev_bquat, s->st.prev_hpos, 1.0f / 30.0f}, obs_cc_args(s, out, zf_mean, zf_std, clip));
+    return launched();
+}
+
 struct Field { int dim; bool view; float* (*row)(const kp_sim&); };
 #define ROW(member) [](const kp_sim& s) -> float* { return s.member; }
 static const Field FIELDS[] = {
@@ -1345,6 +1379,23 @@
     if (obj7 && !row_obj_qpos) return fail("kp_sim_reset_rows: obj7 needs row_obj_qpos");
     HIP_OK(hipSetDevice(s->device));
     if (row_obj_qpos && launch_set_objects(s, "kp_sim_reset_rows", row_obj_qpos, mask, row, row_action_one_hot, obj7)) return -1;
+    if (mask && s->model->boundary_fused) {
+        ResetList& rl = s->rl;
+        unsigned seen = (unsigned)s->n;
+        if (rl.host) { const unsigned v = *(volatile unsigned*)rl.host; seen = std::min(v, seen); }
+        const int rows = (int)std::min<unsigned>((unsigned)s->n, std::max(512u, 2u * seen + 64u));
+        hipLaunchKernelGGL(kp::k_reset_rows_list, dim3((s->n + kp::RESET_SPAN - 1) / kp::RESET_SPAN), dim3(256), 0, s->stream, s->n, init_qpos, init_qvel, row, mask, cur_t,
+                           s->st.qpos, s->st.qvel, s->st.qpos_d, s->st.qvel_d, s->st.warm, aux_rows, aux_rows ? aux_cols : 0, rl.list, rl.cnt + rl.turn, rl.cnt + (rl.turn ^ 1));
+        HIP_OK(hipGetLastError());
+        int rc = launch_step(s, nullptr, 0, nullptr, false, nullptr, rows);
+        if (!rc && set_target) {
+            hipLaunchKernelGGL(kp::k_target_fk_list, dim3((rows + 3) / 4), dim3(256), 0, s->stream, s->n, s->st.qpos, rl.list, rl.cnt + rl.turn, s->tgt,
+                               s->T.body_pos, s->T.body_ipos, s->T.body_parent, s->T.body_depth);
+            rc = launched();
+        }
+        rl.turn ^= 1;
+        return rc;
+    }
     hipLaunchKernelGGL(kp::k_reset_rows, dim3(s->n), dim3(128), 0, s->stream, s->n, init_qpos, init_qvel, row, mask, cur_t, s->st.qpos, s->st.qvel, s->st.qpos_d, s->st.qvel_d,
                        s->st.warm, aux_rows, aux_rows ? aux_cols : 0);
     HIP_OK(hipGetLastError());
diff --git a/kinpoly_amd/csrc/kp_step_kernel.hpp b/kinpoly_amd/csrc/kp_step_kernel.hpp
--- a/kinpoly_amd/csrc/kp_step_kernel.hpp
+++ b/kinpoly_amd/csrc/kp_step_kernel.hpp
@@ -341,6 +341,16 @@
 }
 template <int NT, bool OBJ>
 __global__ __launch_bounds__(NT, (NT == 64 ? 2 : 1)) void kp_forward_kernel(StepArgs A) { step_body<NT, OBJ, true>((int)blockIdx.x, -1); }
+template <int NT, bool OBJ>
+__global__ __launch_bounds__(NT, (NT == 64 ? 2 : 1)) void kp_forward_list_kernel(StepArgs A, const int* __restrict__ list, const unsigned* __restrict__ cnt, unsigned* host_cnt) {
+    const unsigned m = min(*cnt, (unsigned)A.n_envs);
+    if (host_cnt && blockIdx.x == 0 && threadIdx.x == 0) *host_cnt = m;
+    for (unsigned i = blockIdx.x; i < m; i += gridDim.x) {
+        const int e = list[i];
+        if (e >= 0) step_body<NT, OBJ, true>(e, -1);
+        __syncthreads();
+    }
+}
 
 template <bool OBJ, bool LEAN, bool XC>
 __device__ __forceinline__ void step_queue_body(const StepArgs& A, const XcArgs* X) {
diff --git a/kinpoly_amd/env.py b/kinpoly_amd/env.py
--- a/kinpoly_amd/env.py
+++ b/kinpoly_amd/env.py
@@ -333,10 +333,13 @@
         if self.ar_mode:
             sim.step_begin()
             sim.set_target(self._ar_frame("ar_qpos"))
+        rs = self.cc_running_state
+        if not self.ar_mode and sim.cc_obs_dim == 784:
+            cc_obs = sim.step_head_obs_cc(a, self._cc_obs, rs.mean, rs.std, rs.clip)
         else:
-            sim.step_head(a)
-        rs = self.cc_running_state
-        cc_obs = sim.obs_cc(self._cc_obs, rs.mean, rs.std, rs.clip)
+            if not self.ar_mode:
+                sim.step_head(a)
+            cc_obs = sim.obs_cc(self._cc_obs, rs.mean, rs.std, rs.clip)
         mean_action = self.mode == "test" or (self.mode == "train" and self.joint_controller)
         with torch.no_grad():
             cc_action = self.cc_policy.select_action(cc_obs, mean_action, self.gen, cc_noise).contiguous()
diff --git a/kinpoly_amd/sim.py b/kinpoly_amd/sim.py
--- a/kinpoly_amd/sim.py
+++ b/kinpoly_amd/sim.py
@@ -229,7 +229,7 @@
     "kp_sim_render": (_I, [_V, _I, _I, _V, _V, _V, _V, _I, _I, _I, _STYLE, _V, _V, _V]),
     "kp_sim_render_ego": (_I, [_V, _I, _I, _V, _V, _V, _V, _V, _V, _V, _V, _I, _I, _I, _I, _STYLE, _I, _I, _V, _V, _V, _V, _V, _V]),
     "kp_sim_step_ctrl": (_I, [_V, _V, _I, _V]), "kp_sim_step_ctrl_base": (_I, [_V, _V, _I, _V, _V]), "kp_sim_step_kin": (_I, [_V, _V, _V]),
-    "kp_sim_step_head": (_I, [_V, _V]), "kp_sim_step_begin": (_I, [_V]),
+    "kp_sim_step_head": (_I, [_V, _V]), "kp_sim_step_head_obs_cc": (_I, [_V, _V, _V, _V, _V, _F]), "kp_sim_step_begin": (_I, [_V]),
     "kp_sim_obs_cc": (_I, [_V, _V, _V, _V, _F]), "kp_sim_obs_cc_ex": (_I, [_V, _V, _V, _V, _F, _V]), "kp_sim_cc_obs_dim": (_I, [_V]),
     "kp_sim_obs_ar": (_I, [_V, _CTX, _V]), "kp_sim_ar_obs_dim": (_I, [_V]),
     "kp_field_dim": (_I, [_I]), "kp_sim_get": (_I, [_V, _I, _V]), "kp_sim_field_device": (_V, [_V, _I]),
@@ -529,6 +529,13 @@
     def step_head(self, kin_action):
         _check(self.L.kp_sim_step_head(self.h, _ptr(kin_action, self.n, KIN_ACTION_DIM)), "kp_sim_step_head")
 
+    def step_head_obs_cc(self, kin_action, out=None, zf_mean=None, zf_std=None, clip=0.0):
+        out = self._new(self.cc_obs_dim) if out is None else out
+        zm, zs = (_dev("ZFilter mean / std", z if z is None or not z.is_contiguous() else z.view(-1), (self.cc_obs_dim,)) for z in (zf_mean, zf_std))
+        _check(self.L.kp_sim_step_head_obs_cc(self.h, _ptr(kin_action, self.n, KIN_ACTION_DIM), _ptr(out, self.n, self.cc_obs_dim), zm, zs, float(clip)),
+               "kp_sim_step_head_obs_cc")
+        return out
+
     def step_kin(self, kin_action, out=None):
         out = self._new(NQ) if out is None else out
         _check(self.L.kp_sim_step_kin(self.h, _ptr(kin_action, self.n, KIN_ACTION_DIM), _ptr(out, self.n, NQ)), "kp_sim_step_kin")
```

Result: no change. 1.416 million (median of 2 runs) (-0.1%).
